# fredrikekre/PartitionedArrays.jl

Measured on AMD Instinct MI355X. Metric: SpMV+halo GB/s (frac of HBM peak), 3D Poisson 27-pt, 1/2/4/8 MI355X, higher is better.
Workload: dtype f64

## Files before the change

### include/pa_hip.h

```cpp
#ifndef PA_HIP_H
#define PA_HIP_H

#include <stdint.h>

#ifdef __cplusplus
extern "C" {
#endif

enum { PA_F32 = 0, PA_F64 = 1, PA_C64 = 2, PA_C128 = 3 };
enum { PA_REPLACE = 0, PA_ADD = 1 };

typedef struct pa_ctx pa_ctx;
typedef struct pa_index pa_index;
typedef struct pa_xchg pa_xchg;
typedef struct pa_vec pa_vec;
typedef struct pa_mat pa_mat;
typedef struct pa_coo pa_coo;

const char* pa_last_error(void);
int pa_version(void);
int pa_device_count(int* count);
int pa_tune(const char* key, int value, int* previous);
#define PA_TUNE_DROP (-2147483647 - 1)
int pa_ctx_tune(pa_ctx* c, const char* key, int value, int* previous);
// ... 22 lines not shown

int pa_xchg_create(pa_ctx* ctx,
                   int32_t n_rcv, const int32_t* parts_rcv,
                   const int32_t* ptrs_rcv, const int32_t* lids_rcv,
                   int32_t n_snd, const int32_t* parts_snd,
                   const int32_t* ptrs_snd, const int32_t* lids_snd,
                   pa_xchg** out);
int pa_xchg_destroy(pa_xchg* xg);

int pa_index_set_gids(pa_index* idx, const int64_t* lid_to_gid);
int pa_add_gids(pa_index* idx, int64_t n, const int64_t* gids, int64_t cap,
                int64_t* new_gids, int64_t* n_new);
int pa_index_to_lids(pa_index* idx, int64_t n, int64_t* ids);

int pa_vec_create(pa_ctx* ctx, int dtype, int64_t n, pa_vec** out);
int pa_vec_destroy(pa_vec* v);
int pa_vec_upload(pa_vec* v, const void* host, int64_t n);
int pa_vec_download(const pa_vec* v, void* host, int64_t n);
int pa_vec_device_ptr(const pa_vec* v, void** out);
int pa_vec_fill(pa_vec* v, const void* s);
int pa_vec_copy(pa_vec* dst, const pa_index* idx_dst,
                const pa_vec* src, const pa_index* idx_src, int same_layout);
#define PA_BCAST_F64 8
#define PA_BCAST_C128 16
int pa_vec_axpby(pa_vec* y, const pa_vec* x, const pa_index* idx,
                 const void* a, int mode, int all_lids);

int pa_mat_from_csc(pa_ctx* ctx, int dtype, int index_bytes,
                    int64_t nrows_lids, int64_t ncols_lids,
                    const void* colptr, const void* rowval, const void* nzval,
                    const pa_index* rows, const pa_index* cols,
                    pa_mat** out);
int pa_mat_from_csr(pa_ctx* ctx, int dtype, int index_bytes, int Bi,
                    int64_t nrows_lids, int64_t ncols_lids,
                    const void* rowptr, const void* colval, const void* nzval,
                    const pa_index* rows, const pa_index* cols,
                    pa_mat** out);
int pa_mat_from_coo(pa_ctx* ctx, int dtype, int index_bytes, int ids_global,
                    int64_t nrows_lids, int64_t ncols_lids, int64_t ncoo,
                    const void* I, const void* J, const void* V,
                    const pa_index* rows, const pa_index* cols,
                    int64_t* csc_nnz, int64_t* colptr_out,
                    int64_t* rowval_out, pa_mat** out);
int pa_mat_from_coo_csr(pa_ctx* ctx, int dtype, int index_bytes, int ids_global, int Bi,
                        int64_t nrows_lids, int64_t ncols_lids, int64_t ncoo,
                        const void* I, const void* J, const void* V,
                        const pa_index* rows, const pa_index* cols, int64_t* nnz,
                        int64_t* rowptr_out, int64_t* colval_out, pa_mat** out);
int pa_mat_from_dcoo_csr(const pa_coo* coo, int ids_global, int Bi, int64_t nrows_lids,
                         int64_t ncols_lids, const pa_index* rows, const pa_index* cols,
                         int64_t* nnz, int64_t* rowptr_out, int64_t* colval_out,
                         pa_mat** out);
int pa_coo_create(pa_ctx* ctx, int dtype, int64_t n, const int64_t* I,
                  const int64_t* J, const void* V, pa_coo** out);
int pa_coo_destroy(pa_coo* coo);
int pa_coo_size(const pa_coo* coo, int64_t* n);
int pa_coo_download(const pa_coo* coo, int64_t* I, int64_t* J, void* V);
int pa_coo_assemble_all(int n, pa_coo* const coo[], const pa_index* const rows[],
                        pa_xchg* const rows_xchg[]);
int pa_mat_from_dcoo(const pa_coo* coo, int ids_global, int64_t nrows_lids,
                     int64_t ncols_lids, const pa_index* rows,
                     const pa_index* cols, int64_t* csc_nnz,
                     int64_t* colptr_out, int64_t* rowval_out, pa_mat** out);
int pa_mat_set_values(pa_mat* A, const void* nzval);
int pa_mat_fillstored(pa_mat* A, const void* v);
int pa_mat_get_values(const pa_mat* A, void* nzval);
int pa_mat_xchg_create(pa_mat* A, int32_t n_rcv, const int32_t* parts_rcv,
                       const int32_t* ptrs_rcv, const int64_t* k_rcv,
                       int32_t n_snd, const int32_t* parts_snd,
                       const int32_t* ptrs_snd, const int64_t* k_snd,
                       pa_xchg** out);
int pa_mat_exchange_all(int n, pa_mat* const A[], pa_xchg* const xg[],
                        int op, int reverse, int zero_sent);
int pa_mat_destroy(pa_mat* A);
int pa_mat_info(const pa_mat* A, int64_t* nrows_owned, int64_t* nnz_owned,
                int64_t* slots, int64_t* nslices, int64_t* nslices_interior);
int pa_mat_format_info(const pa_mat* A, int64_t* pattern_slices,
                       int64_t* regular_rows, int64_t* side_rows,
                       int64_t* side_slots);
int pa_mat_delta16_info(const pa_mat* A, int64_t* delta16_slices);
int pa_mat_triple_info(const pa_mat* A, int64_t* t_slices, int64_t* t_rows, int64_t* tri_slices,
                       int64_t* tri_rows);
int pa_mat_pair_info(const pa_mat* A, int64_t* pair_slices, int64_t* pair_rows);

int pa_mat_device_ptrs(const pa_mat* A, uint64_t out[8]);

int pa_mat_traffic(const pa_mat* A, int64_t* value_bytes, int64_t* index_bytes,
                   int64_t* meta_bytes);

int pa_mat_long_rows(const pa_mat* A, int64_t* n_long, int64_t* n_long_nnz);

int pa_spmv_all(int n, pa_mat* const A[], pa_vec* const y[],
                const pa_index* const y_idx[],
                pa_vec* const x[], const pa_index* const x_idx[],
                pa_xchg* const xg[], const void* alpha, const void* beta);

int pa_spmv_dot_all(int n, pa_mat* const A[], pa_vec* const y[],
                    const pa_index* const y_idx[],
                    pa_vec* const x[], const pa_index* const x_idx[],
                    pa_xchg* const xg[], const void* alpha, const void* beta,
                    void* dot_result);
int pa_cg_update_all(int n, pa_vec* const x[], pa_vec* const r[],
                     const pa_vec* const u[], const pa_vec* const c[],
                     const pa_index* const idx[], const void* alpha,
                     double* rnorm);

int pa_cg_solve_all(int n, pa_mat* const A[], pa_vec* const x[],
                    const pa_vec* const b[], pa_vec* const u[],
                    pa_vec* const r[], pa_vec* const c[],
                    const pa_index* const idx[], pa_xchg* const xg[],
                    double reltol, double abstol, int64_t maxiter, int batch,
                    int64_t* iterations, double* residual, double* history);

typedef int (*pa_allreduce_max_fn)(float* v, int n, void* user);
int pa_cg_variant_agree(const float local_ms[2], pa_allreduce_max_fn fn, void* user, int* choice);
int pa_cg_fuse_agree(int local_can_fuse, pa_allreduce_max_fn fn, void* user, int* agreed);
int pa_mat_cg_choice(const pa_mat* A, int* choice);

int pa_exchange_all(int n, pa_vec* const v[], pa_xchg* const xg[],
                    const pa_index* const idx[], int op, int reverse,
                    int zero_ghosts);

int pa_dot_all(int n, const pa_vec* const a[], const pa_index* const ia[],
               const pa_vec* const b[], const pa_index* const ib[],
               void* result);
int pa_norm2_all(int n, const pa_vec* const a[], const pa_index* const ia[],
                 void* result);
int pa_sum_all(int n, const pa_vec* const a[], const pa_index* const ia[],
               void* result);

int pa_mat_stencil(pa_ctx* ctx, int dtype, int kind, const int64_t gdims[3],
                   const int64_t box_lo[3], const int64_t box_n[3],
                   int64_t nlids_cols, const int32_t* shell_lid,
                   const double* coeffs, int ncoeffs, pa_mat** out);

int pa_ctx_set_timing(pa_ctx* ctx, int enable);
int pa_ctx_kernel_times(pa_ctx* ctx, float* interior_ms, float* halo_ms,
                        float* boundary_ms, int* count);
int pa_ctx_last_kernel_ms(pa_ctx* ctx, float* spmv_interior_ms,
                          float* spmv_boundary_ms);
int pa_ctx_span(pa_ctx* ctx, int stop);
int pa_ctx_span_ms(pa_ctx* ctx, float* ms);

#ifdef __cplusplus
}
#endif
#endif
```

### partitionedarrays.jl_amd/_lib.py

```python
from __future__ import annotations

import ctypes as C
import os

import numpy as np

_HERE = os.path.dirname(os.path.abspath(__file__))
LIB_PATH = os.environ.get("PA_HIP_LIB") or os.path.join(_HERE, "libpa_hip.so")

PA_F32, PA_F64, PA_C64, PA_C128 = 0, 1, 2, 3
PA_REPLACE, PA_ADD = 0, 1
TUNE_DROP = -(2 ** 31)
PA_BCAST_F64, PA_BCAST_C128 = 8, 16

DTYPES = {
    np.dtype(np.float32): PA_F32,
    np.dtype(np.float64): PA_F64,
    np.dtype(np.complex64): PA_C64,
    np.dtype(np.complex128): PA_C128,
}
NP_OF = {v: k for k, v in DTYPES.items()}

_lib = None
_p = C.c_void_p
_i32p = C.POINTER(C.c_int32)
_i64p = C.POINTER(C.c_int64)

_SIGS = {
    "pa_version": [],
    "pa_device_count": [C.POINTER(C.c_int)],
    "pa_tune": [C.c_char_p, C.c_int, C.POINTER(C.c_int)],
    "pa_ctx_tune": [_p, C.c_char_p, C.c_int, C.POINTER(C.c_int)],
    "pa_knob_selftest": [C.c_int, C.c_int, C.POINTER(C.c_int)],
    "pa_cg_variant_agree": [C.POINTER(C.c_float), _p, _p, C.POINTER(C.c_int)],
    "pa_cg_fuse_agree": [C.c_int, _p, _p, C.POINTER(C.c_int)],
    "pa_mat_cg_choice": [_p, C.POINTER(C.c_int)],
    "pa_hbm_probe": [C.c_int, C.c_int64, C.c_int, C.POINTER(C.c_double), C.POINTER(C.c_double)],
    "pa_issue_stats": [C.c_int, C.POINTER(C.c_double), C.POINTER(C.c_double), C.POINTER(C.c_int64)],
    "pa_hbm_probe_launch": [C.c_int, C.c_int64, C.c_int64, C.c_int, C.POINTER(C.c_double)],
    "pa_ctx_create": [C.c_int, C.c_int, C.c_int, C.POINTER(_p)],
    "pa_ctx_create_shared": [C.c_int, C.c_int, _p, C.POINTER(_p)],
    "pa_ctx_destroy": [_p],
    "pa_ctx_sync": [_p],
    "pa_comm_unique_id": [C.c_char_p],
    "pa_comm_init_rank": [_p, C.c_char_p],
    "pa_comm_init_all": [C.c_int, C.POINTER(_p)],
    "pa_comm_stats": [_p, _i64p, _i64p],
    "pa_comm_info": [_p, C.POINTER(C.c_int), C.POINTER(C.c_int), C.POINTER(C.c_int), C.c_char_p, C.c_int,
                     C.POINTER(C.c_int), C.c_char_p, C.c_int],
    "pa_index_create": [_p, C.c_int64, C.c_int64, _i32p, C.c_int64, _i32p, C.POINTER(_p)],
    "pa_index_destroy": [_p],
    "pa_xchg_create": [_p, C.c_int32, _i32p, _i32p, _i32p, C.c_int32, _i32p, _i32p, _i32p, C.POINTER(_p)],
    "pa_xchg_destroy": [_p],
    "pa_vec_create": [_p, C.c_int, C.c_int64, C.POINTER(_p)],
    "pa_vec_destroy": [_p],
    "pa_vec_upload": [_p, _p, C.c_int64],
    "pa_vec_download": [_p, _p, C.c_int64],
    "pa_vec_device_ptr": [_p, _p],
    "pa_vec_fill": [_p, _p],
    "pa_vec_copy": [_p, _p, _p, _p, C.c_int],
    "pa_vec_axpby": [_p, _p, _p, _p, C.c_int, C.c_int],
    "pa_mat_from_csc": [_p, C.c_int, C.c_int, C.c_int64, C.c_int64, _p, _p, _p, _p, _p, C.POINTER(_p)],
    "pa_mat_from_csr": [_p, C.c_int, C.c_int, C.c_int, C.c_int64, C.c_int64, _p, _p, _p, _p, _p, C.POINTER(_p)],
    "pa_coo_create": [_p, C.c_int, C.c_int64, _i64p, _i64p, _p, C.POINTER(_p)],
    "pa_coo_destroy": [_p],
    "pa_coo_size": [_p, _i64p],
    "pa_coo_download": [_p, _i64p, _i64p, _p],
    "pa_coo_assemble_all": [C.c_int, C.POINTER(_p), C.POINTER(_p), C.POINTER(_p)],
    "pa_mat_from_dcoo": [_p, C.c_int, C.c_int64, C.c_int64, _p, _p, _i64p, _i64p, _i64p, C.POINTER(_p)],
    "pa_mat_from_coo": [_p, C.c_int, C.c_int, C.c_int, C.c_int64, C.c_int64, C.c_int64, _p, _p, _p, _p, _p, _i64p,
                        _i64p, _i64p, C.POINTER(_p)],
    "pa_mat_from_coo_csr": [_p, C.c_int, C.c_int, C.c_int, C.c_int, C.c_int64, C.c_int64, C.c_int64, _p, _p, _p, _p,
                            _p, _i64p, _i64p, _i64p, C.POINTER(_p)],
    "pa_mat_from_dcoo_csr": [_p, C.c_int, C.c_int, C.c_int64, C.c_int64, _p, _p, _i64p, _i64p, _i64p,
                             C.POINTER(_p)],
    "pa_mat_fillstored": [_p, _p],
    "pa_index_set_gids": [_p, _i64p],
    "pa_add_gids": [_p, C.c_int64, _i64p, C.c_int64, _i64p, _i64p],
    "pa_index_to_lids": [_p, C.c_int64, _i64p],
    "pa_mat_set_values": [_p, _p],
    "pa_mat_get_values": [_p, _p],
    "pa_mat_xchg_create": [_p, C.c_int32, _i32p, _i32p, _i64p, C.c_int32, _i32p, _i32p, _i64p, C.POINTER(_p)],
    "pa_mat_exchange_all": [C.c_int, C.POINTER(_p), C.POINTER(_p), C.c_int, C.c_int, C.c_int],
    "pa_mat_destroy": [_p],
    "pa_mat_info": [_p, _i64p, _i64p, _i64p, _i64p, _i64p],
    "pa_mat_format_info": [_p, _i64p, _i64p, _i64p, _i64p],
    "pa_mat_delta16_info": [_p, _i64p],
    "pa_mat_triple_info": [_p, _i64p, _i64p, _i64p, _i64p],
    "pa_mat_pair_info": [_p, _i64p, _i64p],
    "pa_mat_long_rows": [_p, _i64p, _i64p],
    "pa_mat_stencil": [_p, C.c_int, C.c_int, _i64p, _i64p, _i64p, C.c_int64, _i32p, C.POINTER(C.c_double), C.c_int, C.POINTER(_p)],
    "pa_spmv_all": [C.c_int, C.POINTER(_p), C.POINTER(_p), C.POINTER(_p), C.POINTER(_p), C.POINTER(_p), C.POINTER(_p), _p, _p],
    "pa_spmv_dot_all": [C.c_int, C.POINTER(_p), C.POINTER(_p), C.POINTER(_p), C.POINTER(_p), C.POINTER(_p), C.POINTER(_p), _p, _p, _p],
    "pa_cg_update_all": [C.c_int, C.POINTER(_p), C.POINTER(_p), C.POINTER(_p), C.POINTER(_p), C.POINTER(_p), _p, C.POINTER(C.c_double)],
    "pa_cg_solve_all": [C.c_int, C.POINTER(_p), C.POINTER(_p), C.POINTER(_p), C.POINTER(_p), C.POINTER(_p),
                        C.POINTER(_p), C.POINTER(_p), C.POINTER(_p), C.c_double, C.c_double, C.c_int64, C.c_int,
                        _i64p, C.POINTER(C.c_double), C.POINTER(C.c_double)],
    "pa_exchange_all": [C.c_int, C.POINTER(_p), C.POINTER(_p), C.POINTER(_p), C.c_int, C.c_int, C.c_int],
    "pa_dot_all": [C.c_int, C.POINTER(_p), C.POINTER(_p), C.POINTER(_p), C.POINTER(_p), _p],
    "pa_norm2_all": [C.c_int, C.POINTER(_p), C.POINTER(_p), _p],
    "pa_sum_all": [C.c_int, C.POINTER(_p), C.POINTER(_p), _p],
    "pa_ctx_last_kernel_ms": [_p, C.POINTER(C.c_float), C.POINTER(C.c_float)],
    "pa_ctx_kernel_times": [_p, C.POINTER(C.c_float), C.POINTER(C.c_float), C.POINTER(C.c_float),
                            C.POINTER(C.c_int)],
    "pa_mat_traffic": [_p, _i64p, _i64p, _i64p],
    "pa_mat_device_ptrs": [_p, _p],
    "pa_ctx_span": [_p, C.c_int],
    "pa_ctx_span_ms": [_p, C.POINTER(C.c_float)],
    "pa_ctx_set_timing": [_p, C.c_int],
}

EXPORTED = sorted(list(_SIGS) + ["pa_last_error"])


class PAError(RuntimeError):
    pass


def _prepare_runtime():
    try:
        import torch
    except Exception:
        pass


def lib():
    global _lib
    if _lib is not None:
        return _lib
    if not os.path.exists(LIB_PATH):
        raise PAError(f"{LIB_PATH} not built: run `python -c 'import __graft_entry__ as g; g.build()'`")
    _prepare_runtime()
    L = C.CDLL(LIB_PATH)
    for name, args in _SIGS.items():
        if os.environ.get("PA_HIP_LIB") and not hasattr(L, name):
            continue
        f = getattr(L, name)
        f.argtypes = args
        f.restype = C.c_int
    L.pa_last_error.argtypes = []
    L.pa_last_error.restype = C.c_char_p
    _lib = L
    return L


def call(name, *args):
    L = lib()
    rc = getattr(L, name)(*args)
    if rc != 0:
        raise PAError(f"{name}: {L.pa_last_error().decode(errors='replace')}")


def device_count() -> int:
    n = C.c_int(0)
    call("pa_device_count", C.byref(n))
    return n.value


def tune(key: str, value: int) -> int:
    prev = C.c_int(0)
    call("pa_tune", key.encode(), int(value), C.byref(prev))
    return prev.value


def knob_selftest(nthreads: int = 4, iters: int = 2000) -> int:
    n = C.c_int(-1)
    call("pa_knob_selftest", int(nthreads), int(iters), C.byref(n))
    return n.value


ALLREDUCE_MAX_FN = C.CFUNCTYPE(C.c_int, C.POINTER(C.c_float), C.c_int, C.c_void_p)

# ... 68 lines not shown
```

### partitionedarrays.jl_amd/csrc/pa_api.cpp

```cpp
#include <dlfcn.h>
#include <hip/hip_runtime.h>
#include <rccl/rccl.h>

#include <algorithm>
#include <chrono>
#include <cmath>
#include <cstdio>
#include <cstdlib>
#include <cstring>
#include <memory>
#include <numeric>
#include <string>
#include <unordered_map>
#include <atomic>
#include <condition_variable>
#include <functional>
#include <mutex>
#include <thread>
#include <vector>

#include "pa_internal.h"

namespace pa {

static thread_local std::string g_err;
void set_error(const std::string& msg) { g_err = msg; }

void launch_spmv_part(int which, int64_t nwork, const int32_t* list, const pa_mat* A, const void* x,
                      void* y, const int32_t* ymap, bool has_alpha, int bmode, const void* alpha,
                      const void* beta, void* dotp, hipStream_t st,
                      const SpmvPart* cgp = nullptr);
void launch_delta16(pa_mat* A, int64_t noids, const int32_t* kind, int32_t* ok, hipStream_t st);
void launch_pattern_detect(pa_mat* A, int64_t noids, int min_pct, int32_t* kind, int32_t* plen, int32_t* pat,
                           uint64_t* mask, int32_t* pghost, int32_t* nirreg, hipStream_t st);
void launch_side_len(pa_mat* A, int64_t n, const int32_t* rows, int32_t* len, int64_t noids,
                     int32_t* sghost, hipStream_t st);
void launch_side_fill(pa_mat* A, const int32_t* rows, const int32_t* len, hipStream_t st);
void launch_fold(int cplx, int nb, const void* in, void* scratch, void* out, unsigned* ticket, hipStream_t st);
void launch_fold_cg_alpha(int dtype, int nb, const void* in, void* scratch, void* out, unsigned* ticket,
                          CGState* cst, hipStream_t st);
void launch_fold_cg_step(int dtype, int nb, const void* in, void* scratch, void* out, unsigned* ticket,
                         CGState* cst, double* history, hipStream_t st);
void launch_cg_xr(int dtype, int64_t n, int64_t noids, const int32_t* own, void* x, void* r, const void* u,
                  const void* c, const void* alpha, const CGState* cst, double* part, int nb, hipStream_t st);
void launch_cg_xu(int dtype, int64_t n, void* x, void* u, const void* r, const CGState* cst, hipStream_t st);
void launch_cg_ghost(int dtype, int64_t lo, int64_t hi, const void* r, const void* uo, void* un, void* x,
                     const CGState* cst, hipStream_t st);
void launch_cg_alpha(int dtype, int P, const void* gathered, CGState* cst, hipStream_t st);
void launch_cg_step(int dtype, int P, const double* gathered, CGState* cst, double* history, hipStream_t st);
void launch_gather_ptrs(int P, const void* const* srcs, int accsz, void* out, hipStream_t st);
void launch_gather_scatter(int P, const void* const* srcs, int accsz, int nd, void* const* dsts, hipStream_t st);
const Knobs kDefaults = {
     223,  1,  1,  1,  1,
     65536,  2,  1,  0,  1,
     1,  0,  1,  0,  -1,  1,
     1,  1,  1,  0,  7,  1};
int coo_compress(int dtype, int index_bytes, int64_t m, int64_t ncols, int64_t n, const void* dI, const void* dJ,
                 const void* dV, int csr, int64_t* nu_out, int32_t** crow, int32_t** ccol, void** cval,
                 int64_t** colptr, hipStream_t st, hipError_t* err_out);
int coo_row_order(int64_t nu, const int32_t* crow, const int32_t* ccol, const int32_t* rl2o, const int32_t* cl2o,
                  int64_t nrows, int64_t noids_c, int64_t ncols, int H, uint64_t** key2, int64_t** idx2,
                  int64_t** rowptr, int64_t** gflag, int64_t** grank, int32_t** slen, int32_t** sghost,
                  int64_t* nnz_out, int64_t* ngh_out, hipStream_t st, hipError_t* err_out);
void coo_slices(int64_t ns, int64_t nrows, int H, const int64_t* rowptr, const uint64_t* key2, int64_t ncols,
                int64_t noids_c, const int32_t* lidx, int32_t* slen, int32_t* sghost, hipStream_t st);
void coo_fill(int dtype, int64_t nnz, int64_t nu, const uint64_t* key2, const int64_t* idx2, const int64_t* rowptr,
              const int64_t* soff, int H, int R, int64_t ncols, const int32_t* ccol, const void* cval,
              const int64_t* gflag, const int64_t* grank, int64_t slots, int32_t* col, void* val, int64_t* nz_slot,
              const int32_t* lidx, const int64_t* lptr, int32_t* lcol, int64_t long_off, hipStream_t st);
void launch_fill_i32(int64_t n, int32_t* a, int32_t v, hipStream_t st);
void launch_spmv_long(const pa_mat* A, const void* x, void* y, const int32_t* ymap, bool has_alpha, int bmode,
                      const void* alpha, const void* beta, void* dotp, int64_t dot_base, hipStream_t st);
int gid_table(int64_t n, const int64_t* d_lid_to_gid, uint64_t** sgid, int64_t** slid, hipStream_t st);
int gids_to_lids(int64_t n, int64_t* ids, const uint64_t* sgid, const int64_t* slid, int64_t nl, hipStream_t st);
int coo_assemble_pack(int dtype, int64_t n, const int64_t* I, const int64_t* J, void* V, const uint64_t* sgid,
                      const int64_t* slid, int64_t nl, const std::vector<int32_t>& lid_to_ohid, int nseg,
                      const int32_t* d_lids_rcv, const std::vector<int64_t>& ptrs_rcv, int64_t** sI, int64_t** sJ,
                      void** sV, std::vector<int64_t>* cnt, hipStream_t st);
int gids_first_touch(int64_t n, const int64_t* gids, const uint64_t* sgid, const int64_t* slid, int64_t nl,
                     int64_t** out, int64_t* m_out, hipStream_t st);
void launch_pack(int dtype, int64_t n, const int32_t* lids, const void* v, void* buf,
                 hipStream_t st, hipEvent_t ev = nullptr);
void launch_unpack(int dtype, int64_t n, const int32_t* lids, const pa_combine_plan& plan, int op,
                   const void* buf, void* v, hipStream_t st);
void launch_pull(int dtype, int64_t n, const int32_t* lids, const pa_combine_plan& plan, int op, const int32_t* bid,
                 const int64_t* elem, const void* const* bases, void* v, hipStream_t st, hipEvent_t ev = nullptr);
void launch_fill(int dtype, int64_t n, int64_t base, const int32_t* map, void* v, const void* s,
                 hipStream_t st);
int launch_spmv_merged(int n, const int* which, const SpmvPart* parts, bool has_alpha, int bmode,
                       const void* alpha, const void* beta, pa_ctx* owner,
                       hipStream_t st);
void launch_spmv_group(int which, int np, const SpmvPart* parts, bool has_alpha, int bmode, const void* alpha,
                       const void* beta, hipStream_t st);
void launch_pack_group(int dtype, const PackGroup& g, hipStream_t st);
void launch_pull_group(int dtype, const PullGroup& g, hipStream_t st);
void launch_copy(int dtype, int64_t n, const int32_t* dmap, void* d, const int32_t* smap,
                 const void* s, hipStream_t st);
void launch_axpby(int dtype, int64_t n, const int32_t* map, void* y, const void* x, const void* a,
                  int mode, hipStream_t st, int sk = 0);
void launch_reduce(int dtype, int kind, int64_t n, const int32_t* ma, const void* a,
                   const int32_t* mb, const void* b, void* partials, void* result,
                   unsigned* ticket, hipStream_t st);
void launch_stencil_count(const StencilGeom& g, const int32_t* shell, const double* coef,
                          int64_t nrows, int noids, int H, int32_t* slen, int32_t* sghost,
                          int32_t* err, hipStream_t st);
void launch_stencil_fill(const StencilGeom& g, const int32_t* shell, const double* coef,
                         int64_t nrows, int noids, pa_mat* A, int32_t* err, hipStream_t st);
void launch_probe(int copy, int unroll, int64_t n16, const void* a, void* b, int blocks, hipStream_t st);
void launch_invalid_config();
void launch_t_rowinfo(const pa_mat* A, int64_t n, const int32_t* rows, int64_t noids, int32_t* info, hipStream_t st);
void launch_t_pairinfo(const pa_mat* A, int64_t n, const int32_t* rows, int32_t* pairable, hipStream_t st);
void launch_u_fill(const pa_mat* A, hipStream_t st);
void launch_t_gbase(const pa_mat* A, int64_t noids, int32_t* ok, hipStream_t st);
void launch_t_fill(const pa_mat* A, int64_t noids, bool codes, hipStream_t st);
void launch_t_check(const pa_mat* A, unsigned* bad, hipStream_t st);

}

using namespace pa;

#define PA_FAIL(msg)             \
  do {                           \
    pa::set_error(msg);          \
    return -1;                   \
  } while (0)

#define HIPC(expr)                                                                       \
  do {                                                                                   \
    hipError_t e_ = (expr);                                                              \
    if (e_ != hipSuccess) {                                                              \
      pa::set_error(std::string(#expr) + " failed: " + hipGetErrorString(e_));           \
      return -1;                                                                         \
    }                                                                                    \
  } while (0)

#define NCCLC(expr)                                                                      \
  do {                                                                                   \
    ncclResult_t r_ = (expr);                                                            \
    if (r_ != ncclSuccess) {                                                             \
      pa::set_error(std::string(#expr) + " failed: " + ncclGetErrorString(r_));          \
      return -1;                                                                         \
    }                                                                                    \
  } while (0)

#define CHECK_ARG(cond, msg) \
  do {                       \
    if (!(cond)) PA_FAIL(msg); \
  } while (0)

namespace {

template <typename T>
int dev_upload(T** dptr, const std::vector<T>& h) {
  *dptr = nullptr;
  if (h.empty()) return 0;
  HIPC(hipMalloc((void**)dptr, h.size() * sizeof(T)));
  HIPC(hipMemcpy(*dptr, h.data(), h.size() * sizeof(T), hipMemcpyHostToDevice));
  return 0;
}

void dev_free(void* p) {
  if (p) (void)hipFree(p);
}

bool valid_dtype(int dt) { return dt == PA_F32 || dt == PA_F64 || dt == PA_C64 || dt == PA_C128; }

bool scalar_is(int dt, const void* s, double re) {
  switch (dt) {
    case PA_F32: return *(const float*)s == (float)re;
    case PA_F64: return *(const double*)s == re;
    case PA_C64: { const float* f = (const float*)s; return f[0] == (float)re && f[1] == 0.f; }
    case PA_C128: { const double* d = (const double*)s; return d[0] == re && d[1] == 0.0; }
  }
  return false;
}

int build_plan(const std::vector<int32_t>& lids, pa_combine_plan* plan) {
  const int64_t n = (int64_t)lids.size();
  std::vector<int32_t> order(n);
  std::iota(order.begin(), order.end(), 0);
  std::stable_sort(order.begin(), order.end(), [&](int32_t a, int32_t b) { return lids[a] < lids[b]; });
  std::vector<int32_t> target, ptr{0}, pos;
  pos.reserve(n);
  for (int64_t i = 0; i < n; ++i) {
    const int32_t l = lids[order[i]];
    if (target.empty() || target.back() != l) {
      if (!target.empty()) ptr.push_back((int32_t)pos.size());
      target.push_back(l);
    }
    pos.push_back(order[i]);
  }
  if (!target.empty()) ptr.push_back((int32_t)pos.size());
  plan->ntargets = (int64_t)target.size();
  plan->unique = plan->ntargets == n;
  if (!plan->unique) {
// ... 47 lines not shown
  cstart.push_back(lptr.back());
  if (dev_upload(&A->d_lchunk_start, cstart) || dev_upload(&A->d_lrow_chunk, rchunk)) return -1;
  HIPC(hipMalloc(&A->d_lpart, std::max<int64_t>(A->n_lchunks, 1) * 16));
  if (!lcol.empty() && dev_upload(&A->d_long_col, lcol)) return -1;
  return 0;
}

inline bool is_long_row(const pa_mat* A, int64_t r) {
  return A->n_long > 0 && std::binary_search(A->h_long_rows.begin(), A->h_long_rows.end(), (int32_t)r);
}

inline int64_t nvals(const pa_mat* A) { return A->slots + A->n_gnz + A->n_lnz; }

int finish_sell_layout(pa_mat* A, const std::vector<int32_t>& slen, const std::vector<char>& sghost,
                       std::vector<int64_t>* soff_out) {
  const int64_t ns = (int64_t)slen.size();
  std::vector<int64_t> soff(ns);
  int64_t acc = 0;
  for (int64_t s = 0; s < ns; ++s) {
    soff[s] = acc;
    acc += (int64_t)slen[s] * A->H;
  }
  A->slots = acc;
  A->nslices = ns;
  A->h_slen = slen;
  A->maxlen_all = 0;
  for (int32_t l : slen) A->maxlen_all = std::max(A->maxlen_all, (int)l);
  std::vector<int32_t> ilist, blist;
  for (int64_t s = 0; s < ns; ++s) (sghost[s] ? blist : ilist).push_back((int32_t)s);
  A->nslices_int = (int64_t)ilist.size();
  if (dev_upload(&A->d_slice_off, soff)) return -1;
  if (dev_upload(&A->d_slice_len, slen)) return -1;
  if (!blist.empty()) {
    if (dev_upload(&A->d_int_list, ilist)) return -1;
    if (dev_upload(&A->d_bnd_list, blist)) return -1;
  }
  if (soff_out) *soff_out = std::move(soff);
  return 0;
}

void free_uniform(pa_mat* A) {
  dev_free(A->d_uval);
  dev_free(A->d_uemap);
  A->d_uval = nullptr;
  A->d_uemap = nullptr;
  A->uK = 0;
}

int build_uniform(pa_mat* A, const std::vector<int32_t>& kind, const std::vector<int32_t>& table,
                  const std::vector<int32_t>& packed, std::vector<int32_t>& desc) {
  free_uniform(A);
  if (!knobs().spmv_uniform || A->dtype != PA_F64 || A->R != 2 || A->npatterns == 0) return 0;
  const int64_t ns = A->nslices, K0 = A->kmax, np = A->npatterns;
  std::vector<int32_t> plen(np, 0);
  for (int64_t s = 0; s < ns; ++s)
    if (kind[s] == 1) plen[packed[s] >> 9] = packed[s] & 0xff;
  std::vector<int32_t> U;
  for (int64_t p = 0; p < np; ++p)
    for (int32_t k = 0; k < plen[p]; ++k) U.push_back(table[p * K0 + k]);
  std::sort(U.begin(), U.end());
  U.erase(std::unique(U.begin(), U.end()), U.end());
  if (U.size() > 7 || U.empty()) return 0;
  const int K = (int)U.size();
  std::vector<int32_t> emap(np * 8, 0), emask(np, 0);
  for (int64_t p = 0; p < np; ++p)
    for (int32_t k = 0; k < plen[p]; ++k) {
      const int e = (int)(std::lower_bound(U.begin(), U.end(), table[p * K0 + k]) - U.begin());
      CHECK_ARG(k == 0 || e > emap[p * 8 + k - 1], "uniform layout: a pattern out of column order (internal error)");
      emap[p * 8 + k] = e;
      emask[p] |= 1 << e;
    }
  const int DW = desc_words(A->R);
  for (int64_t s = 0; s < ns; ++s)
    if (kind[s] == 1) desc[DW * s + 2] = emask[packed[s] >> 9];
  hipStream_t st = A->ctx->s_main;
  const size_t S = dtype_size(A->dtype);
  if (dev_upload(&A->d_uemap, emap)) return -1;
  HIPC(hipMalloc(&A->d_uval, (size_t)ns * A->H * K * S));
  HIPC(hipMemsetAsync(A->d_uval, 0, (size_t)ns * A->H * K * S, st));
  A->uK = K;
  for (int e = 0; e < 8; ++e) A->upat[e] = e < K ? U[e] : 0;
  launch_u_fill(A, st);
  HIPC(hipGetLastError());
  return 0;
}

int dedup_patterns(pa_mat* A, const std::vector<int32_t>& kind) {
  const int64_t ns = A->nslices, K = A->kmax;
  hipStream_t st = A->ctx->s_main;
  std::vector<int32_t> pat(ns * K);
  HIPC(hipMemcpyAsync(pat.data(), A->d_pat, ns * K * 4, hipMemcpyDeviceToHost, st));
  HIPC(hipStreamSynchronize(st));
  std::vector<int32_t> table, packed(A->h_plen);
  std::unordered_map<std::string, int32_t> ids;
  int64_t reach = 0;
  for (int64_t s = 0; s < ns; ++s) {
    if (kind[s] != 1) continue;
    const int32_t len = A->h_plen[s];
    CHECK_ARG(len >= 1 && len <= 255, "pattern slice with more than 255 entries per row");
    std::string key(reinterpret_cast<const char*>(&pat[s * K]), (size_t)len * 4);
    auto it = ids.find(key);
    int32_t id;
    if (it == ids.end()) {
      id = (int32_t)ids.size();
      CHECK_ARG(id < (1 << 22), "more than 2^22 distinct slice patterns");
      ids.emplace(std::move(key), id);
      table.insert(table.end(), pat.begin() + s * K, pat.begin() + (s + 1) * K);
      for (int32_t k = 0; k < len; ++k) reach = std::max<int64_t>(reach, std::llabs((long long)pat[s * K + k]));
    } else {
      id = it->second;
    }
    bool tri = len % 3 == 0;
    for (int32_t k = 0; tri && k < len; k += 3)
      tri = pat[s * K + k + 1] == pat[s * K + k] + 1 && pat[s * K + k + 2] == pat[s * K + k] + 2;
    packed[s] = len | ((tri ? 1 : 0) << 8) | (id << 9);
  }
  A->npatterns = (int64_t)ids.size();
  A->xcd_auto = (int)std::min<int64_t>(64, reach / (4 * A->H) / 8);
  dev_free(A->d_pat);
  A->d_pat = nullptr;
  if (table.empty()) table.assign(K, 0);
  if (dev_upload(&A->d_pat, table)) return -1;
  HIPC(hipMemcpyAsync(A->d_plen, packed.data(), ns * 4, hipMemcpyHostToDevice, st));
  {
    std::vector<int64_t> soff(ns);
    HIPC(hipMemcpyAsync(soff.data(), A->d_slice_off, ns * 8, hipMemcpyDeviceToHost, st));
    HIPC(hipStreamSynchronize(st));
    const int W = A->H / 64, DW = desc_words(A->R);
    std::vector<uint64_t> mask(ns * W);
    HIPC(hipMemcpyAsync(mask.data(), A->d_mask, ns * W * 8, hipMemcpyDeviceToHost, st));
    HIPC(hipStreamSynchronize(st));
    std::vector<int32_t> desc(DW * ns, 0);
    for (int64_t s = 0; s < ns; ++s) {
      CHECK_ARG(soff[s] % A->H == 0 && soff[s] / A->H <= INT32_MAX, "slice offset outside the descriptor's range");
      desc[DW * s] = (int32_t)(soff[s] / A->H);
      desc[DW * s + 1] = packed[s];
      std::memcpy(&desc[DW * s + 4], &mask[s * W], W * 8);
    }
    if (build_uniform(A, kind, table, packed, desc)) return -1;
    dev_free(A->d_pdesc);
    A->d_pdesc = nullptr;
    if (dev_upload(&A->d_pdesc, desc)) return -1;
  }
  HIPC(hipStreamSynchronize(st));
  return 0;
}

int remap_nz_interleaved(pa_mat* A, const std::vector<int32_t>& kind, hipStream_t st) {
  HIPC(hipStreamSynchronize(st));
  if (A->d_nz_slot) {
    A->h_nz_slot.resize(A->csc_nnz);
    HIPC(hipMemcpy(A->h_nz_slot.data(), A->d_nz_slot, A->csc_nnz * 8, hipMemcpyDeviceToHost));
    dev_free(A->d_nz_slot);
    A->d_nz_slot = nullptr;
  }
  const int64_t ns = A->nslices, R = A->R, H = A->H;
  std::vector<int64_t> soff(ns);
  HIPC(hipMemcpy(soff.data(), A->d_slice_off, ns * 8, hipMemcpyDeviceToHost));
  for (int64_t& slot : A->h_nz_slot) {
    if (slot < 0) continue;
    const int64_t s = (int64_t)(std::upper_bound(soff.begin(), soff.end(), slot) - soff.begin()) - 1;
    if (kind[s] != 3) continue;
    const int64_t t = slot - soff[s], k = t / H, w = t % H;
    slot = soff[s] + (k * 64 + w % 64) * R + w / 64;
  }
  return 0;
// ... 231 lines not shown
    HIPC(hipStreamSynchronize(st));
    dev_free(d_ok);
    int64_t nd = 0;
    for (int64_t s = 0; s < ns; ++s)
      if (ok[s]) { kind[s] = 3; ++nd; }
    if (nd == 0) {
      dev_free(A->d_col16);
      dev_free(A->d_gbase);
      A->d_col16 = nullptr;
      A->d_gbase = nullptr;
    } else {
      HIPC(hipMemcpyAsync(A->d_kind, kind.data(), ns * 4, hipMemcpyHostToDevice, st));
      if (A->nz_map && A->R == 4 && remap_nz_interleaved(A, kind, st)) return -1;
      if (knobs().spmv_tri16 && A->R <= 2 && build_triple_sell(A, kind, noids)) return -1;
    }
  }
  std::vector<int32_t> pint, pbnd, xint, xbnd, dint, dbnd, side;
  for (int64_t s = 0; s < ns; ++s) {
    if (kind[s] == 1) (pghost[s] ? pbnd : pint).push_back((int32_t)s);
    else if (kind[s] == 3) (pghost[s] ? dbnd : dint).push_back((int32_t)s);
    else if (kind[s] == 0) (pghost[s] ? xbnd : xint).push_back((int32_t)s);
    if (kind[s] == 1) {
      ++A->npattern_slices;
      const int64_t nvalid = std::min<int64_t>(A->H, A->nrows - s * A->H);
      for (int64_t i = 0; i < nvalid; ++i) {
        if ((mask[s * W + i / 64] >> (i & 63)) & 1ull) ++A->nregular_rows;
        else if (!is_long_row(A, s * A->H + i)) side.push_back((int32_t)(s * A->H + i));
      }
    }
  }
  A->h_kind = kind;
  A->maxlen_pat = A->maxlen_pm_int = A->maxlen_d16 = 0;
  for (int64_t s = 0; s < ns; ++s) {
    if (kind[s] == 1) A->maxlen_pat = std::max(A->maxlen_pat, (int)A->h_plen[s]);
    else if (kind[s] == 0) A->maxlen_pm_int = std::max(A->maxlen_pm_int, (int)A->h_slen[s]);
    else if (kind[s] == 3) A->maxlen_d16 = std::max(A->maxlen_d16, (int)A->h_slen[s]);
  }
  A->np_int = (int64_t)pint.size();
  A->np_bnd = (int64_t)pbnd.size();
  A->nx_int = (int64_t)xint.size();
  A->nx_bnd = (int64_t)xbnd.size();
  A->nd_int = (int64_t)dint.size();
  A->nd_bnd = (int64_t)dbnd.size();
  if (dev_upload(&A->d_pint_list, pint) || dev_upload(&A->d_pbnd_list, pbnd) ||
      dev_upload(&A->d_xint_list, xint) || dev_upload(&A->d_xbnd_list, xbnd) ||
      dev_upload(&A->d_dint_list, dint) || dev_upload(&A->d_dbnd_list, dbnd))
    return -1;
  A->s_nrows = (int64_t)side.size();
  std::vector<int32_t> rl;
  if (A->s_nrows > 0) {
    if (dev_upload(&A->d_s_rowmap, side)) return -1;
    int32_t* srow = A->d_s_rowmap;
    int32_t* d_dummy = nullptr;
    A->s_nslices = (A->s_nrows + A->H - 1) / A->H;
    HIPC(hipMalloc((void**)&A->d_s_rowlen, A->s_nrows * 4));
    HIPC(hipMalloc((void**)&d_dummy, A->s_nslices * 4));
    HIPC(hipMemsetAsync(d_dummy, 0, A->s_nslices * 4, st));
    launch_side_len(A, A->s_nrows, srow, A->d_s_rowlen, noids, d_dummy, st);
    HIPC(hipGetLastError());
    rl.resize(A->s_nrows);
    HIPC(hipMemcpyAsync(rl.data(), A->d_s_rowlen, A->s_nrows * 4, hipMemcpyDeviceToHost, st));
    HIPC(hipStreamSynchronize(st));
    dev_free(d_dummy);
  }
  if (A->s_nrows > 0) {
    int32_t* srow = A->d_s_rowmap;
    std::vector<int32_t> slen(A->s_nslices, 0);
    std::vector<int64_t> soff(A->s_nslices);
    for (int64_t i = 0; i < A->s_nrows; ++i) slen[i / A->H] = std::max(slen[i / A->H], rl[i]);
    A->maxlen_side = 0;
    for (int32_t l : slen) A->maxlen_side = std::max(A->maxlen_side, (int)l);
    int64_t acc = 0;
    for (int64_t s = 0; s < A->s_nslices; ++s) { soff[s] = acc; acc += (int64_t)slen[s] * A->H; }
    A->s_slots = acc;
    if (dev_upload(&A->d_s_off, soff) || dev_upload(&A->d_s_len, slen)) return -1;
    const size_t S = dtype_size(A->dtype);
    HIPC(hipMalloc((void**)&A->d_s_col, std::max<int64_t>(acc, 1) * 4));
    HIPC(hipMalloc(&A->d_s_val, std::max<int64_t>(acc, 1) * S));
    launch_side_fill(A, srow, A->d_s_rowlen, st);
    HIPC(hipGetLastError());
    HIPC(hipStreamSynchronize(st));
  }
  A->has_pat = true;
  return 0;
}

struct LocalSet {
  std::vector<int> pos_of_part;
  int find(int part) const {
    return (part >= 1 && part < (int)pos_of_part.size()) ? pos_of_part[part] : -1;
  }
};

template <typename H>
LocalSet local_set(int n, H* const* hs) {
  LocalSet L;
  int maxp = 0;
  bool all_comm = true;
  for (int i = 0; i < n; ++i) {
    const pa_ctx* c = hs[i]->ctx;
    maxp = std::max(maxp, c->nparts);
    all_comm = all_comm && c->comm != nullptr && (c->halo_rccl || knobs().halo_transport == 1);
  }
  L.pos_of_part.assign(maxp + 1, -1);
  if (all_comm) return L;
  for (int i = 0; i < n; ++i) L.pos_of_part[hs[i]->ctx->part] = i;
  return L;
}

uint64_t g_xchg_next_id = 1;

int build_pull(int i, int n, pa_xchg* const xg[], const LocalSet& L, int dtype, int dir, bool alt = false) {
  pa_xchg* X = xg[i];
  pa_ctx* c = X->ctx;
  pa_pull& P = alt ? X->pull_alt : X->pull[dir];
  auto sender_buf = [&](const pa_xchg* Q) -> void* {
    return alt ? Q->d_buf_snd2 : (dir == 0 ? Q->d_buf_snd : Q->d_buf_rcv);
  };
  const auto& prcv = dir == 0 ? X->parts_rcv : X->parts_snd;
  const auto& orcv = dir == 0 ? X->ptrs_rcv : X->ptrs_snd;
  void* own = dir == 0 ? X->d_buf_rcv : X->d_buf_snd;
  std::vector<const void*> key;
  key.push_back((const void*)(intptr_t)dtype_size(dtype));
  for (int32_t q : prcv) {
    const int j = L.find(q);
    key.push_back(j >= 0 ? (const void*)(uintptr_t)xg[j]->id : nullptr);
    key.push_back(j >= 0 ? sender_buf(xg[j]) : own);
  }
  if (P.built && P.key == key) return 0;
  dev_free(P.d_bid);
  dev_free(P.d_elem);
  dev_free(P.d_bases);
  P = pa_pull{};
  P.built = true;
  P.key = key;
  HIPC(hipSetDevice(c->device));
  std::vector<void*> bases;
  auto base_id = [&](void* b) {
    for (size_t t = 0; t < bases.size(); ++t)
      if (bases[t] == b) return (int32_t)t;
    bases.push_back(b);
    return (int32_t)(bases.size() - 1);
  };
  const int64_t nslots = orcv.empty() ? 0 : orcv.back();
  std::vector<int32_t> bid(nslots);
  std::vector<int64_t> elem(nslots);
  for (size_t k = 0; k < prcv.size(); ++k) {
    const int j = L.find(prcv[k]);
    const int64_t cnt = orcv[k + 1] - orcv[k];
    if (j < 0) {
      const int32_t b = base_id(own);
      for (int64_t t = 0; t < cnt; ++t) { bid[orcv[k] + t] = b; elem[orcv[k] + t] = orcv[k] + t; }
      continue;
    }
    pa_xchg* Q = xg[j];
    const auto& qsnd = dir == 0 ? Q->parts_snd : Q->parts_rcv;
    const auto& qo = dir == 0 ? Q->ptrs_snd : Q->ptrs_rcv;
    int m = -1;
    for (size_t t = 0; t < qsnd.size(); ++t)
      if (qsnd[t] == c->part) { m = (int)t; break; }
    CHECK_ARG(m >= 0, "exchanger mismatch: a receiver lists a sender that does not send to it");
    CHECK_ARG(cnt == qo[m + 1] - qo[m], "exchanger mismatch: segment lengths differ (SequentialBackend.jl:187)");
    const int qdev = Q->ctx->device;
    if (qdev != c->device) {
      int can = 0;
      HIPC(hipDeviceCanAccessPeer(&can, c->device, qdev));
// ... 374 lines not shown
  const Knobs* kn_ = nullptr;
  int n_ = 0;
  std::vector<std::thread> workers_;
};

}

static std::shared_ptr<void> own_comm(ncclComm_t comm) {
  return std::shared_ptr<void>((void*)comm, [](void* p) { (void)ncclCommDestroy((ncclComm_t)p); });
}

extern "C" {

const char* pa_last_error(void) { return g_err.c_str(); }
int pa_version(void) { return 1; }

}
namespace {
struct Knob {
  const char* key;
  int Knobs::*slot;
  int64_t Knobs::*slot64;
  int64_t lo, hi;
  int64_t mask;
  const char* help;
};
const Knob kKnobs[] = {
    {"spmv_flags", &Knobs::spmv_flags, nullptr, 0, 0xff, 0xff,
     "spmv_flags: bit 0 = non-temporal streams, bit 1 = pattern and triple-SELL slices' one-load descriptor, "
     "bit 2 = 16 B x runs (pattern rows), bit 3 = masked tail batch, bit 4 = identity slice lists dropped, "
     "bit 5 = non-temporal y stores, bit 6 = short-row kernels (launches whose rows have <= 8 entries), "
     "bit 7 = the Float64 short-row tail launch at 7 entries and 7 waves per SIMD (rows <= 7 entries)"},
    {"long_rows_exact", &Knobs::long_exact, nullptr, 0, 1, 0,
     "long_rows_exact: 1 = reference summation order, 0 = lane-strided tree (1e-12)"},
    {"halo_pull", &Knobs::halo_pull, nullptr, 0, 1, 0,
     "halo_pull: 1 = receivers read the senders' buffers (one kernel), 0 = staging copies"},
    {"spmv_delta16", &Knobs::spmv_delta16, nullptr, 0, 1, 0,
     "spmv_delta16: 1 = int32-column slices whose columns fit 16-bit codes store those (matrices built "
     "afterwards; default), 0 = int32 column ids"},
    {"spmv_merge", &Knobs::spmv_merge, nullptr, 0, 1, 0,
     "spmv_merge: 1 = mul! without a halo in flight (one part, or parts of one stream pair with the direct "
     "pull) runs every slice kind of every part as one launch (default), 0 = one launch per kind"},
    {"spmv_merge_max", nullptr, &Knobs::spmv_merge_max, 0, INT32_MAX, 0,
     "spmv_merge_max: one part with more slices than this runs one launch per kind (0: always merge)"},
    {"cg_fuse", &Knobs::cg_fuse, nullptr, 0, 2, 0,
     "cg_fuse: 1 = the device CG computes u = r .+ beta.*u inside the SpMV, 0 = a separate sweep, "
     "2 = auto (default: one batch of each, then the faster; all parts in one process, else the sweep)"},
    {"halo_direct", &Knobs::halo_direct, nullptr, 0, 1, 0,
     "halo_direct: 1 = mul! over parts sharing a stream pair reads the ghosts straight from the owners' x "
     "on the compute stream (default), 0 = pack + pull on the comm stream"},
    {"halo_transport", &Knobs::halo_transport, nullptr, 0, 1, 0,
     "halo_transport: 0 = parts of this process by device reads/copies, 1 = RCCL send/recv for every part "
     "with a communicator (pa_comm_init_all)"},
    {"spmv_group", &Knobs::spmv_group, nullptr, 0, 1, 0,
     "spmv_group: 1 = one launch per phase for parts sharing a stream pair, 0 = per part"},
    {"spmv_format", &Knobs::spmv_format, nullptr, 0, 1, 0, "spmv_format: 0 = int32 columns, 1 = pattern slices"},
    {"pattern_min_regular", &Knobs::pattern_min_pct, nullptr, 0, 100, 0,
     "pattern_min_regular: a slice becomes a pattern slice when at least this % of its rows follow its pattern "
     "(matrices built afterwards); 0 = auto (default): 70 for 128-row slices, 50 for Float32's 256-row slices"},
    {"issue_threads", &Knobs::issue_threads, nullptr, 0, 2, 0,
     "issue_threads: a call over parts with their own stream pairs is issued from host threads, one part "
     "per thread: 1 = when the parts span several devices (default), 2 = always, 0 = never (the calling "
     "thread, one part after the other)"},
    {"spmv_tri16", &Knobs::spmv_tri16, nullptr, 0, 1, 0,
     "spmv_tri16: the delta16 slices' rows re-sliced into the triple SELL (rows of consecutive column triples "
     "keep one 16-bit code per triple; matrices built afterwards): 1 = slices of 1-2 rows per lane (Float64, "
     "ComplexF32, ComplexF64, Float32 with f32_rows 2; default), 0 = never"},
    {"f32_rows", &Knobs::f32_rows, nullptr, 0, 4, 6,
     "f32_rows: Float32 SELL rows per lane (matrices built afterwards): 4 = 16 B value packs in 256-row "
     "slices, 2 = 8 B packs in 128-row slices (the Float64 geometry; delta16 rows then take the triple "
     "SELL), 0 = auto (default): 4, rebuilt with 2 when fewer than 80 % of the slices are pattern slices "
     "(C5 F32 -7 %, FE27 256^3 F32 +14 % with 2, profiles/r05/af/)"},
    {"spmv_tri_pack", &Knobs::tri_pack, nullptr, 0, 7, 0,
     "spmv_tri_pack: triple-SELL slices of 2 rows per lane (matrices built afterwards): bit 2 = pair slices "
     "(all element types): rows a, a + 1 whose columns differ by one, entry for entry, share one lane, one "
     "code and one x run per triple (C5 F32 -2.4 %, F64 -1 %, profiles/r06/u/); bit 0 = Float32 pair slices: "
     "a triple's values as one 16 B pack (entries 0 and 1 of both rows) and one 8 B pack (entry 2) per lane "
     "(two loads instead of three); bit 1: unused since r06/aa (the Float32 tri slices' code packs); 7 = "
     "default, 0 = none"},
    {"spmv_uniform", &Knobs::spmv_uniform, nullptr, 0, 1, 0,
     "spmv_uniform: Float64 pattern slices whose patterns (<= 7 entries) fit one union U (FD7; matrices built "
     "afterwards): 1 = a copy of their values at slice * H * |U| in U's entry order, so the short-row tail "
     "launch issues its value and x loads before the slice descriptor arrives (default), 0 = off"},
    {"spmv_side_tail", &Knobs::side_tail, nullptr, 0, 1, 0,
     "spmv_side_tail: per-kind launches without a halo in flight (big single parts): 1 = the side rows (<= 8 "
     "entries) run as the trailing waves of the pattern launch (default: FE27 256^3 -0.4 %, profiles/r05/o/), "
     "0 = a launch of their own after it"},
    {"spmv_tri_order", &Knobs::tri_order, nullptr, 0, 1, 0,
     "spmv_tri_order: the triple SELL's row order (matrices built afterwards): 1 = the other rows first "
     "(their slower waves start early, the launch ends on uniform triple slices; default: C5 F64 -1 %, "
     "Float32 triples -4..-7 %, profiles/r05/n/), 0 = rows of column triples first"},
    {"halo_barrier", &Knobs::halo_barrier, nullptr, 0, 2, 0,
     "halo_barrier: mul! over parts with their own stream pairs and local neighbours (one process driving "
     "several GPUs): 1 = one pack barrier event per call and double-buffered send buffers (default), 2 = the "
     "same with each part's pull on its compute stream after its interior slices (one runtime call less per "
     "part), 0 = per-neighbour event waits before every pack and every pull"},
    {"spmv_xcd_chunk", &Knobs::spmv_xcd_chunk, nullptr, -1, 64, 0,
     "spmv_xcd_chunk: the SpMV launches' workgroups in runs of C consecutive blocks per XCD (C > 0; the x lines "
     "of neighbouring slices shared in one L2), 0 = the hardware's round robin, -1 = auto (default): per-kind "
     "launches (big single parts) take C = the pattern's reach in blocks / 8, so that a block's z-neighbour "
     "plane runs on its XCD (FE27 256^3 F64: C = 16, -1.0..-1.2 %, profiles/r05/q,r/), merged launches keep "
     "the round robin (C2: C = 4 +1.4 %, r05/k/)"},
    {"fault_inject", &Knobs::fault_inject, nullptr, 0, 1, 0,
     "fault_inject: 1 = every job of a threaded issue (IssuePool) also issues an invalid kernel launch (tests "
     "of the error path; test_exception.jl's role), 0 = off (default)"},
};
constexpr int kNumKnobs = (int)(sizeof(kKnobs) / sizeof(kKnobs[0]));
static_assert(kNumKnobs <= pa_ctx::kMaxKnobs, "pa_ctx::over too small");

std::mutex g_knob_mu;
Knobs g_knob_defaults = kDefaults;
thread_local const Knobs* t_knobs = nullptr;
thread_local Knobs t_knob_snapshot;

int knob_find(const char* key) {
  for (int i = 0; i < kNumKnobs; ++i)
    if (!std::strcmp(key, kKnobs[i].key)) return i;
  pa::set_error(std::string("pa_tune: unknown key ") + key);
  return -1;
}
int knob_index(const char* key, int64_t value) {
  const int i = knob_find(key);
  if (i < 0) return -1;
  const Knob& k = kKnobs[i];
  if (value < k.lo || value > k.hi || (k.mask != 0 && (value & ~k.mask) != 0)) {
    pa::set_error(k.help);
    return -2;
  }
  return i;
}
int64_t knob_get(const Knobs& K, int i) { return kKnobs[i].slot ? (int64_t)(K.*kKnobs[i].slot) : K.*kKnobs[i].slot64; }
void knob_set(Knobs& K, int i, int64_t v) {
  if (kKnobs[i].slot) K.*kKnobs[i].slot = (int)v;
  else K.*kKnobs[i].slot64 = v;
}
}

namespace pa {
const Knobs& knobs() {
  if (t_knobs) return *t_knobs;
  std::lock_guard<std::mutex> g(g_knob_mu);
  t_knob_snapshot = g_knob_defaults;
  return t_knob_snapshot;
}
KnobBind::KnobBind(const Knobs* k) : prev(t_knobs) { t_knobs = k; }
KnobBind::~KnobBind() { t_knobs = prev; }
thread_local int t_force_f32_rows = 0;
int f32_rows_knob() { return t_force_f32_rows ? t_force_f32_rows : (knobs().f32_rows == 2 ? 2 : 4); }
struct ForceF32Rows {
  int prev;
  explicit ForceF32Rows(int r) : prev(t_force_f32_rows) { t_force_f32_rows = r; }
  ~ForceF32Rows() { t_force_f32_rows = prev; }
};
}

TuneScope::TuneScope(const pa_ctx* c) : prev(t_knobs) {
  if (prev) {
    k = *prev;
  } else {
    std::lock_guard<std::mutex> g(g_knob_mu);
    k = g_knob_defaults;
  }
  if (c && !prev)
    for (int i = 0; i < kNumKnobs; ++i)
      if (c->has_over[i]) knob_set(k, i, c->over[i]);
  t_knobs = &k;
// ... 1302 lines not shown
      const int64_t k = std::find(qr.begin(), qr.end(), c->part) - qr.begin();
      const Side& src = sd[jj];
      const int64_t from = src.off[k];
      const int sdev = xg[jj]->ctx->device;
      if (sdev == c->device) {
        HIPC(hipMemcpyAsync(d.nI + at, src.sI + from, m * 8, hipMemcpyDeviceToDevice, c->s_main));
        HIPC(hipMemcpyAsync(d.nJ + at, src.sJ + from, m * 8, hipMemcpyDeviceToDevice, c->s_main));
        HIPC(hipMemcpyAsync((char*)d.nV + at * S, (const char*)src.sV + from * S, m * S, hipMemcpyDeviceToDevice,
                            c->s_main));
      } else {
        HIPC(hipMemcpyPeerAsync(d.nI + at, c->device, src.sI + from, sdev, m * 8, c->s_main));
        HIPC(hipMemcpyPeerAsync(d.nJ + at, c->device, src.sJ + from, sdev, m * 8, c->s_main));
        HIPC(hipMemcpyPeerAsync((char*)d.nV + at * S, c->device, (const char*)src.sV + from * S, sdev, m * S,
                                c->s_main));
      }
    }
    for (size_t k = 0; k < X->parts_rcv.size(); ++k) {
      const int64_t m = d.cnt[k];
      const int q = X->parts_rcv[k];
      if (m == 0 || L.find(q) >= 0) continue;
      const int pr = c->peer_rank(q);
      ncclComm_t cm = (ncclComm_t)c->comm;
      ops.push_back({c->part, q, true, (char*)(d.sI + d.off[k]), (size_t)m * 8, pr, cm, c->s_main});
      ops.push_back({c->part, q, true, (char*)(d.sJ + d.off[k]), (size_t)m * 8, pr, cm, c->s_main});
      ops.push_back({c->part, q, true, (char*)d.sV + d.off[k] * S, (size_t)m * S, pr, cm, c->s_main});
    }
  }
  if (!ops.empty() && rccl_group(ops)) { free_all(); return -1; }
  for (int i = 0; i < n; ++i) {
    HIPC(hipSetDevice(coo[i]->ctx->device));
    HIPC(hipStreamSynchronize(coo[i]->ctx->s_main));
  }
  for (int i = 0; i < n; ++i) {
    pa_coo* C = coo[i];
    Side& d = sd[i];
    HIPC(hipSetDevice(C->ctx->device));
    dev_free(C->d_I);
    dev_free(C->d_J);
    dev_free(C->d_V);
    C->d_I = d.nI;
    C->d_J = d.nJ;
    C->d_V = d.nV;
    C->n = d.nn;
    d.nI = nullptr;
    d.nJ = nullptr;
    d.nV = nullptr;
  }
  free_all();
  return 0;
}

static int load_nz_map(const pa_mat* cA) {
  CHECK_ARG(cA->nz_map, "matrix was not built from a CSC pattern");
  pa_mat* A = const_cast<pa_mat*>(cA);
  if (A->d_nz_slot) {
    HIPC(hipSetDevice(A->ctx->device));
    HIPC(hipStreamSynchronize(A->ctx->s_main));
    A->h_nz_slot.resize(A->csc_nnz);
    HIPC(hipMemcpy(A->h_nz_slot.data(), A->d_nz_slot, A->csc_nnz * 8, hipMemcpyDeviceToHost));
    dev_free(A->d_nz_slot);
    A->d_nz_slot = nullptr;
  }
  return 0;
}

static inline int64_t nz_index(const pa_mat* A, int64_t p) {
  const int64_t s = A->h_nz_slot[p];
  return s >= 0 ? s : A->slots - s - 1;
}

static int refresh_side(pa_mat* A, hipStream_t st) {
  if (A->s_nrows > 0) {
    launch_side_fill(A, A->d_s_rowmap, A->d_s_rowlen, st);
    HIPC(hipGetLastError());
  }
  if (A->t_nrows > 0) {
    launch_t_fill(A, 0, false, st);
    HIPC(hipGetLastError());
  }
  if (A->d_uval) {
    launch_u_fill(A, st);
    HIPC(hipGetLastError());
  }
  return 0;
}

int pa_mat_set_values(pa_mat* A, const void* nzval) {
  CHECK_ARG(A && nzval, "null argument");
  if (load_nz_map(A)) return -1;
  HIPC(hipSetDevice(A->ctx->device));
  const size_t S = dtype_size(A->dtype);
  const int64_t nv = nvals(A);
  std::vector<unsigned char> hval(nv * S, 0);
  for (int64_t p = 0; p < A->csc_nnz; ++p)
    std::memcpy(&hval[nz_index(A, p) * S], (const unsigned char*)nzval + p * S, S);
  HIPC(hipStreamSynchronize(A->ctx->s_main));
  if (nv) HIPC(hipMemcpy(A->d_val, hval.data(), nv * S, hipMemcpyHostToDevice));
  if (refresh_side(A, A->ctx->s_main)) return -1;
  HIPC(hipStreamSynchronize(A->ctx->s_main));
  return 0;
}

int pa_mat_fillstored(pa_mat* A, const void* v) {
  CHECK_ARG(A && v, "null argument");
  HIPC(hipSetDevice(A->ctx->device));
  const int64_t nv = nvals(A);
  if (nv) launch_fill(A->dtype, nv, 0, nullptr, A->d_val, v, A->ctx->s_main);
  HIPC(hipGetLastError());
  if (refresh_side(A, A->ctx->s_main)) return -1;
  return 0;
}

int pa_mat_get_values(const pa_mat* A, void* nzval) {
  CHECK_ARG(A && nzval, "null argument");
  if (load_nz_map(A)) return -1;
  HIPC(hipSetDevice(A->ctx->device));
  const size_t S = dtype_size(A->dtype);
  const int64_t nv = nvals(A);
  std::vector<unsigned char> hval(nv * S, 0);
  HIPC(hipStreamSynchronize(A->ctx->s_comm));
  HIPC(hipStreamSynchronize(A->ctx->s_main));
  if (nv) HIPC(hipMemcpy(hval.data(), A->d_val, nv * S, hipMemcpyDeviceToHost));
  for (int64_t p = 0; p < A->csc_nnz; ++p)
    std::memcpy((unsigned char*)nzval + p * S, &hval[nz_index(A, p) * S], S);
  return 0;
}

int pa_mat_xchg_create(pa_mat* A, int32_t n_rcv, const int32_t* parts_rcv, const int32_t* ptrs_rcv,
                       const int64_t* k_rcv, int32_t n_snd, const int32_t* parts_snd, const int32_t* ptrs_snd,
                       const int64_t* k_snd, pa_xchg** out) {
  CHECK_ARG(A && out, "null argument");
  if (load_nz_map(A)) return -1;
  CHECK_ARG(nvals(A) < ((int64_t)1 << 31), "matrix exchanger: value index exceeds int32");
  CHECK_ARG(n_rcv >= 0 && n_snd >= 0, "negative neighbour count");
  auto conv = [&](int32_t n, const int32_t* ptrs, const int64_t* k, std::vector<int32_t>& o) -> int {
    const int64_t m = n > 0 ? (int64_t)ptrs[n] - 1 : 0;
    CHECK_ARG(m >= 0, "matrix exchanger: bad ptrs");
    o.resize(m);
    for (int64_t i = 0; i < m; ++i) {
      CHECK_ARG(k[i] >= 1 && k[i] <= A->csc_nnz, "matrix exchanger: nz index out of range");
      o[i] = (int32_t)(nz_index(A, k[i] - 1) + 1);
    }
    return 0;
  };
  std::vector<int32_t> lr, ls;
  if (conv(n_rcv, ptrs_rcv, k_rcv, lr) || conv(n_snd, ptrs_snd, k_snd, ls)) return -1;
  return pa_xchg_create(A->ctx, n_rcv, parts_rcv, ptrs_rcv, lr.data(), n_snd, parts_snd, ptrs_snd, ls.data(),
                        out);
}

int pa_mat_exchange_all(int n, pa_mat* const A[], pa_xchg* const xg[], int op, int reverse, int zero_sent) {
  CHECK_ARG(n >= 1 && A && xg && A[0], "null argument");
  TuneScope ts(A[0]->ctx);
  std::vector<pa_vec> vs(n);
  std::vector<pa_vec*> vp(n);
  for (int i = 0; i < n; ++i) {
    CHECK_ARG(A[i] && xg[i] && A[i]->ctx == xg[i]->ctx, "exchange!(A): matrix and exchanger of different parts");
    vs[i].ctx = A[i]->ctx;
    vs[i].dtype = A[i]->dtype;
    vs[i].n = nvals(A[i]);
    vs[i].d = A[i]->d_val;
    vp[i] = &vs[i];
  }
  if (pa_exchange_all(n, vp.data(), xg, nullptr, op, reverse, 0)) return -1;
  for (int i = 0; i < n; ++i) {
    pa_ctx* c = A[i]->ctx;
    HIPC(hipSetDevice(c->device));
    if (zero_sent) {
      unsigned char z[16] = {0};
      if (reverse) launch_fill(A[i]->dtype, xg[i]->n_rcv_data, 0, xg[i]->d_lids_rcv, A[i]->d_val, z, c->s_main);
      else launch_fill(A[i]->dtype, xg[i]->n_snd_data, 0, xg[i]->d_lids_snd, A[i]->d_val, z, c->s_main);
    }
    if (refresh_side(A[i], c->s_main)) return -1;
  }
  HIPC(hipGetLastError());
  return 0;
}

int pa_mat_destroy(pa_mat* A) {
  if (!A) return 0;
  (void)hipSetDevice(A->ctx->device);
  (void)hipStreamSynchronize(A->ctx->s_main);
  dev_free(A->d_slice_off);
  dev_free(A->d_slice_len);
  dev_free(A->d_int_list);
  dev_free(A->d_bnd_list);
  dev_free(A->d_col);
  dev_free(A->d_val);
  dev_free(A->d_nz_slot);
  for (void* p : {(void*)A->d_kind, (void*)A->d_plen, (void*)A->d_pdesc, (void*)A->d_pat, (void*)A->d_mask,
                  (void*)A->d_pint_list, (void*)A->d_pbnd_list, (void*)A->d_xint_list,
                  (void*)A->d_xbnd_list, (void*)A->d_s_off, (void*)A->d_s_len,
                  (void*)A->d_s_col, A->d_s_val, (void*)A->d_s_rowmap, (void*)A->d_s_rowlen, A->d_dotp,
                  (void*)A->d_long_row, (void*)A->d_long_ptr, (void*)A->d_long_col, (void*)A->d_sflags,
                  (void*)A->d_lmask, (void*)A->d_lchunk_start, (void*)A->d_lrow_chunk, A->d_lpart,
                  (void*)A->d_col16, (void*)A->d_gbase, (void*)A->d_dint_list, (void*)A->d_dbnd_list})
    dev_free(p);
  free_triple_sell(A);
  free_uniform(A);
  delete A;
  return 0;
}

int pa_mat_format_info(const pa_mat* A, int64_t* pattern_slices, int64_t* regular_rows,
                       int64_t* side_rows, int64_t* side_slots) {
  CHECK_ARG(A, "null matrix");
  if (pattern_slices) *pattern_slices = A->npattern_slices;
  if (regular_rows) *regular_rows = A->nregular_rows;
  if (side_rows) *side_rows = A->s_nrows;
  if (side_slots) *side_slots = A->s_slots;
  return 0;
}

int pa_mat_delta16_info(const pa_mat* A, int64_t* delta16_slices) {
  CHECK_ARG(A, "null matrix");
  if (delta16_slices) *delta16_slices = A->nd_int + A->nd_bnd;
  return 0;
}

int pa_mat_pair_info(const pa_mat* A, int64_t* pair_slices, int64_t* pair_rows) {
  CHECK_ARG(A, "null matrix");
  if (pair_slices) *pair_slices = A->t_pair_slices;
  if (pair_rows) *pair_rows = A->t_pair_rows;
  return 0;
}

int pa_mat_triple_info(const pa_mat* A, int64_t* t_slices, int64_t* t_rows, int64_t* tri_slices,
                       int64_t* tri_rows) {
  CHECK_ARG(A, "null matrix");
  if (t_slices) *t_slices = A->t_nslices;
  if (t_rows) *t_rows = A->t_nrows;
  if (tri_slices) *tri_slices = A->t_tri_slices;
  if (tri_rows) *tri_rows = A->t_tri_rows;
  return 0;
}

int pa_mat_long_rows(const pa_mat* A, int64_t* n_long, int64_t* n_long_nnz) {
  CHECK_ARG(A, "null matrix");
  if (n_long) *n_long = A->n_long;
  if (n_long_nnz) *n_long_nnz = A->n_lnz;
  return 0;
}

int pa_mat_device_ptrs(const pa_mat* A, uint64_t out[8]) {
  CHECK_ARG(A && out, "null argument");
  const void* p[8] = {A->d_val, A->d_col, A->d_slice_off, A->d_plen, A->d_pat, A->d_mask, A->d_s_val, A->d_s_col};
  for (int i = 0; i < 8; ++i) out[i] = (uint64_t)(uintptr_t)p[i];
  return 0;
}

int pa_mat_traffic(const pa_mat* A, int64_t* value_bytes, int64_t* index_bytes, int64_t* meta_bytes) {
  CHECK_ARG(A, "null matrix");
  TuneScope ts(A->ctx);
  const int64_t S = (int64_t)dtype_size(A->dtype), H = A->H, W = H / 64;
  const bool pat = knobs().spmv_format == 1 && A->has_pat;
  const bool split = A->d_bnd_list != nullptr;
  int64_t v = 0, ix = 0, m = 0;
  for (int64_t s = 0; s < A->nslices; ++s) {
    const int kd = pat ? A->h_kind[s] : 0;
    if (kd == 1) {
      v += (int64_t)(A->d_uval ? A->uK : A->h_plen[s]) * H * S;
      m += std::max<int64_t>(W * 8 + 8 + 4, 4 * desc_words(A->R)) + 4;
    } else if (kd == 3) {
      v += (int64_t)A->h_slen[s] * H * S;
      ix += (int64_t)A->h_slen[s] * H * 2;
      m += 8 + 4 + 4 + 4;
    } else if (kd == 5) {
    } else {
      v += (int64_t)A->h_slen[s] * H * S;
      ix += (int64_t)A->h_slen[s] * H * 4;
      m += 8 + 4 + ((pat || split) ? 4 : 0);
    }
  }
  if (pat) {
    m += A->npatterns * A->kmax * 4;
    v += A->s_slots * S;
    ix += A->s_slots * 4 + A->s_nrows * 4;
    m += A->s_nslices * 12;
    v += A->t_slots * S;
    ix += A->t_code_slots * 2 + A->t_nrows * 4;
    m += A->t_nslices * (8 + 4 + 4 + 4);
  }
  v += A->n_lnz * S;
  ix += A->n_lnz * 4;
  m += A->n_long * 16;
  if (value_bytes) *value_bytes = v;
  if (index_bytes) *index_bytes = ix;
  if (meta_bytes) *meta_bytes = m;
  return 0;
}

int pa_mat_info(const pa_mat* A, int64_t* nrows, int64_t* nnz, int64_t* slots, int64_t* nslices,
                int64_t* nslices_int) {
  CHECK_ARG(A, "null matrix");
  if (nrows) *nrows = A->nrows;
  if (nnz) *nnz = A->nnz;
  if (slots) *slots = A->slots;
  if (nslices) *nslices = A->nslices;
  if (nslices_int) *nslices_int = A->nslices_int;
  return 0;
}

constexpr int kMaxTimed = 1024;

struct CGFuse {
  std::vector<const void*> u_old;
  std::vector<void*> u_new, xacc;
  std::vector<CGState*> st;
};

static void cg_ghosts(const CGFuse* fz, int i, const pa_mat* A, const pa_vec* r, hipStream_t st) {
  if (!fz || r->n <= A->nrows) return;
  launch_cg_ghost(A->dtype, A->nrows, r->n, r->d, fz->u_old[i], fz->u_new[i], fz->xacc[i], fz->st[i], st);
}

static int group_ok(int n, pa_mat* const A[], pa_xchg* const xg[], bool any_x, int dt) {
  if (!knobs().spmv_group || (n < 2 && any_x)) return 0;
  const pa_ctx* c0 = A[0]->ctx;
  for (int i = 0; i < n; ++i)
    if (A[i]->ctx->s_main != c0->s_main || A[i]->ctx->s_comm != c0->s_comm) return 0;
  if (!any_x) return 1;
  if (!knobs().halo_pull) return 0;
  LocalSet L = local_set(n, xg);
  for (int i = 0; i < n; ++i)
    for (const auto* lst : {&xg[i]->parts_snd, &xg[i]->parts_rcv})
      for (int32_t q : *lst)
        if (L.find(q) < 0) return 0;
  for (int i = 0; i < n; ++i)
    if (!xg[i]->plan_fwd.unique) return 0;
  if (knobs().halo_direct) {
    bool ok = true;
    for (int i = 0; i < n && ok; ++i) {
      if (build_direct(i, n, xg, L)) return 0;
      ok = xg[i]->direct.ok;
    }
    if (ok) return 2;
  }
  for (int i = 0; i < n; ++i) {
    if (build_pull(i, n, xg, L, dt, 0)) return 0;
    if (!xg[i]->pull[0].ok) return 0;
  }
  return 1;
}
// ... 1148 lines not shown
```

### partitionedarrays.jl_amd/csrc/pa_internal.h

```cpp
#pragma once
#include <hip/hip_runtime.h>
#include <cstdint>
#include <memory>
#include <string>
#include <vector>

#include "../../include/pa_hip.h"

namespace pa {

struct alignas(8) c64 {
  float re, im;
};
struct alignas(16) c128 {
  double re, im;
};

__host__ __device__ inline c64 operator+(c64 a, c64 b) { return {a.re + b.re, a.im + b.im}; }
__host__ __device__ inline c64 operator-(c64 a, c64 b) { return {a.re - b.re, a.im - b.im}; }
__host__ __device__ inline c64 operator*(c64 a, c64 b) {
  return {a.re * b.re - a.im * b.im, a.re * b.im + a.im * b.re};
}
__host__ __device__ inline c128 operator+(c128 a, c128 b) { return {a.re + b.re, a.im + b.im}; }
__host__ __device__ inline c128 operator-(c128 a, c128 b) { return {a.re - b.re, a.im - b.im}; }
// ... 185 lines not shown
  int np;
  int64_t n[PA_GROUP_MAX];
  const int32_t* lids[PA_GROUP_MAX];
  const void* v[PA_GROUP_MAX];
  void* buf[PA_GROUP_MAX];
};
struct PullGroup {
  int np;
  int64_t n[PA_GROUP_MAX];
  const int32_t* lids[PA_GROUP_MAX];
  const int32_t* bid[PA_GROUP_MAX];
  const int64_t* elem[PA_GROUP_MAX];
  const void* const* bases[PA_GROUP_MAX];
  void* v[PA_GROUP_MAX];
};

struct StencilGeom {
  int64_t N[3];
  int64_t lo[3];
  int64_t n[3];
  int kind;
};

}

struct pa_ctx {
  struct StreamRefs { int n = 1; };
  StreamRefs* stream_refs = nullptr;
  int device = 0;
  int part = 1;
  int nparts = 1;
  hipStream_t s_main = nullptr;
  hipStream_t s_comm = nullptr;
  void* comm = nullptr;
  bool halo_rccl = false;
  std::shared_ptr<void> comm_owner;
  std::shared_ptr<const std::vector<int>> rank_of_part;
  int peer_rank(int q) const { return rank_of_part ? (*rank_of_part)[q - 1] : q - 1; }
  int64_t rccl_bytes_sent = 0, rccl_bytes_recv = 0;
  void* d_partials = nullptr;
  void* d_fold = nullptr;
  void* d_result = nullptr;
  void* d_gather = nullptr;
  unsigned* d_ticket = nullptr;
  void* h_pinned = nullptr;
  bool timing = false;
  std::vector<hipEvent_t> tev;
  int tn = 0;
  hipEvent_t span_ev[2] = {nullptr, nullptr};
  hipEvent_t ev_packed = nullptr;
  hipEvent_t ev_recvd = nullptr;
  hipEvent_t ev_barrier = nullptr;
  std::vector<std::pair<std::vector<void*>, void**>> bases_cache;
  std::vector<std::pair<std::vector<char>, void*>> merged_cache;
  static constexpr int kMaxKnobs = 24;
  bool has_over[kMaxKnobs] = {};
  int64_t over[kMaxKnobs] = {};
};

namespace pa {
struct Knobs {
  int spmv_flags;
  int long_exact;
  int halo_pull;
  int spmv_delta16;
  int spmv_merge;
  int64_t spmv_merge_max;
  int cg_fuse;
  int halo_direct;
  int halo_transport;
  int spmv_group;
  int spmv_format;
  int pattern_min_pct;
  int issue_threads;
  int fault_inject;
  int spmv_xcd_chunk;
  int spmv_tri16;
  int halo_barrier;
  int tri_order;
  int side_tail;
  int f32_rows;
  int tri_pack;
  int spmv_uniform;
};
const Knobs& knobs();
struct KnobBind {
  explicit KnobBind(const Knobs* k);
  ~KnobBind();
  const Knobs* prev;
};
}

struct TuneScope {
  explicit TuneScope(const pa_ctx* c);
  ~TuneScope();
  TuneScope(const TuneScope&) = delete;
  TuneScope& operator=(const TuneScope&) = delete;
  pa::Knobs k;
  const pa::Knobs* prev;
};

struct pa_index {
  pa_ctx* ctx = nullptr;
  int64_t nlids = 0, noids = 0, nhids = 0;
  bool own_contig = true;
  bool ghost_contig = true;
  int32_t* d_oid_to_lid = nullptr;
  int32_t* d_hid_to_lid = nullptr;
  std::vector<int32_t> h_oid_to_lid;
  std::vector<int32_t> h_hid_to_lid;
  std::vector<int32_t> h_lid_to_ohid;
  uint64_t* d_sgid = nullptr;
  int64_t* d_slid = nullptr;
  bool has_gids = false;
};

struct pa_combine_plan {
  int64_t ntargets = 0;
  bool unique = true;
  int32_t* d_target = nullptr;
  int32_t* d_ptr = nullptr;
  int32_t* d_pos = nullptr;
};

struct pa_pull {
  bool built = false;
  bool ok = false;
  std::vector<const void*> key;
  int32_t* d_bid = nullptr;
  int64_t* d_elem = nullptr;
  void** d_bases = nullptr;
  std::vector<int32_t> h_bid;
  std::vector<int64_t> h_elem;
  std::vector<void*> h_bases;
};

struct pa_xchg {
  pa_ctx* ctx = nullptr;
  uint64_t id = 0;
  pa_pull pull[2];
  pa_pull direct;
  std::vector<int32_t> h_lids_snd;
  std::vector<int32_t> parts_rcv, parts_snd;
  std::vector<int64_t> ptrs_rcv, ptrs_snd;
  int64_t n_rcv_data = 0, n_snd_data = 0;
  int64_t max_lid = -1;
  int32_t* d_lids_rcv = nullptr;
  int32_t* d_lids_snd = nullptr;
  void* d_buf_rcv = nullptr;
  void* d_buf_snd = nullptr;
  void* d_buf_snd2 = nullptr;
  pa_pull pull_alt;
  uint64_t fast_key = 0, fast_seq = 0;
  int fast_parity = 0;
  pa_combine_plan plan_fwd;
  pa_combine_plan plan_rev;
};

constexpr size_t kVecPad = 64;

struct pa_coo {
  pa_ctx* ctx = nullptr;
  int dtype = PA_F64;
  int64_t n = 0;
  int64_t* d_I = nullptr;
  int64_t* d_J = nullptr;
// ... 10 lines not shown

constexpr int desc_words(int R) { return R <= 2 ? 8 : 16; }

struct pa_mat {
  pa_ctx* ctx = nullptr;
  int dtype = PA_F64;
  int cg_fuse_choice = -1;
  int R = 2;
  int H = 128;
  int64_t nrows = 0;
  int64_t ncols_lids = 0;
  int64_t nnz = 0;
  int64_t slots = 0;
  int64_t nslices = 0;
  int64_t nslices_int = 0;
  bool csr = false;
  std::vector<int32_t> h_slen;
  std::vector<int32_t> h_kind;
  std::vector<int32_t> h_plen;
  int maxlen_all = INT32_MAX, maxlen_pm_int = INT32_MAX, maxlen_pat = INT32_MAX, maxlen_side = INT32_MAX;
  int64_t* d_slice_off = nullptr;
  int32_t* d_slice_len = nullptr;
  int32_t* d_int_list = nullptr;
  int32_t* d_bnd_list = nullptr;
  int32_t* d_col = nullptr;
  void* d_val = nullptr;
  std::vector<int64_t> h_nz_slot;
  int64_t* d_nz_slot = nullptr;
  bool nz_map = false;
  int64_t csc_nnz = 0;
  int64_t n_gnz = 0;
  int64_t n_long = 0, n_lnz = 0, long_off = 0;
  int32_t* d_long_row = nullptr;
  int64_t* d_long_ptr = nullptr;
  int32_t* d_long_col = nullptr;
  int32_t* d_sflags = nullptr;
  uint64_t* d_lmask = nullptr;
  std::vector<int32_t> h_long_rows;
  int64_t n_lchunks = 0;
  int64_t* d_lchunk_start = nullptr;
  int64_t* d_lrow_chunk = nullptr;
  void* d_lpart = nullptr;

  bool has_pat = false;
  int kmax = 0;
  int32_t* d_kind = nullptr;
  int32_t* d_pdesc = nullptr;
  int32_t* d_plen = nullptr;
  int32_t* d_pat = nullptr;
  int64_t npatterns = 0;
  int xcd_auto = 0;
  uint64_t* d_mask = nullptr;
  int32_t* d_pint_list = nullptr;
  int32_t* d_pbnd_list = nullptr;
  int64_t np_int = 0, np_bnd = 0;
  int32_t* d_xint_list = nullptr;
  int32_t* d_xbnd_list = nullptr;
  int64_t nx_int = 0, nx_bnd = 0;
  int64_t npattern_slices = 0, nregular_rows = 0;
  uint16_t* d_col16 = nullptr;
  int32_t* d_gbase = nullptr;
  int32_t* d_dint_list = nullptr;
  int32_t* d_dbnd_list = nullptr;
  int64_t nd_int = 0, nd_bnd = 0;
  int maxlen_d16 = INT32_MAX;
  int64_t s_nrows = 0, s_nslices = 0, s_slots = 0;
  int64_t* d_s_off = nullptr;
  int32_t* d_s_len = nullptr;
  int32_t* d_s_col = nullptr;
  void* d_s_val = nullptr;
  int32_t* d_s_rowmap = nullptr;
  int32_t* d_s_rowlen = nullptr;
  int64_t t_nrows = 0, t_nslices = 0, t_slots = 0, t_tri_slices = 0, t_tri_rows = 0, t_code_slots = 0;
  int64_t* d_t_off = nullptr;
  int32_t* d_t_len = nullptr;
  uint16_t* d_t_col16 = nullptr;
  void* d_t_val = nullptr;
  int t_pack = 0;
  int64_t t_pair_slices = 0, t_pair_rows = 0;
  void* d_uval = nullptr;
  int32_t* d_uemap = nullptr;
  int uK = 0;
  int32_t upat[8] = {0, 0, 0, 0, 0, 0, 0, 0};
  int32_t* d_t_gbase = nullptr;
  int32_t* d_t_desc = nullptr;
  int32_t* d_t_rowmap = nullptr;
  int64_t* d_t_src = nullptr;
  int32_t* d_t_rowlen = nullptr;
  int32_t* d_t_int_list = nullptr;
  int32_t* d_t_bnd_list = nullptr;
  int64_t nt_int = 0, nt_bnd = 0;
  int maxlen_t = INT32_MAX;
  std::vector<int32_t> h_t_len;
  void* d_dotp = nullptr;
};
```

### partitionedarrays.jl_amd/csrc/pa_spmv.hip

```cpp
#include "pa_internal.h"

#include <cstddef>

#include <algorithm>
#include <cstring>
#include <type_traits>

#if defined(PA_SPMV_DT)
#define PA_DT_DEFINE 0
#else
#define PA_DT_DEFINE 1
#endif
#define PA_CAT2(a, b) a##b
#define PA_CAT(a, b) PA_CAT2(a, b)

namespace pa {

template <typename T, int R>
struct alignas(sizeof(T) * R) Pack {
  T v[R];
};
template <int R>
struct alignas(4 * R) IPack {
  int32_t c[R];
};
template <int R>
struct alignas(2 * R) S16Pack {
  uint16_t c[R];
};

enum { SPMV_NT = 1, SPMV_DESC = 2 , SPMV_XPAIR = 4, SPMV_TAILB = 8, SPMV_IDLIST = 16, SPMV_YNT = 32, SPMV_SHORT = 64,
       SPMV_SHORT7 = 128 ,
       SPMV_PRODA = 256 ,
       SPMV_TPACK = 512  };

typedef unsigned int spmv_u32x4 __attribute__((ext_vector_type(4)));
static_assert((SPMV_NT | SPMV_DESC | SPMV_XPAIR | SPMV_TAILB | SPMV_IDLIST | SPMV_SHORT | SPMV_SHORT7) == 223,
              "kDefaults.spmv_flags");
template <int R>
constexpr int kDescWords = desc_words(R);

#if defined(__HIP_DEVICE_COMPILE__)
#define PA_GLB __attribute__((address_space(1)))
#else
#define PA_GLB
#endif

template <int BYTES> struct RawOf;
template <> struct RawOf<2> { typedef unsigned short type; };
template <> struct RawOf<4> { typedef unsigned int type; };
template <> struct RawOf<8> { typedef unsigned int type __attribute__((ext_vector_type(2))); };
template <> struct RawOf<16> { typedef unsigned int type __attribute__((ext_vector_type(4))); };

template <bool NT, typename V>
__device__ __forceinline__ V ld(const V* p) {
  typedef typename RawOf<sizeof(V)>::type Raw;
  Raw r;
  if (NT) r = __builtin_nontemporal_load(reinterpret_cast<const Raw*>(p));
  else r = *reinterpret_cast<const Raw*>(p);
  V v;
  __builtin_memcpy(&v, &r, sizeof(V));
  return v;
}

template <typename T>
struct SpmvArgs {
  int64_t nwork;
  const PA_GLB int32_t* list;
  const PA_GLB int64_t* soff;
  const PA_GLB int32_t* slen;
  const PA_GLB int32_t* col;
  const PA_GLB T* val;
  const PA_GLB int32_t* pat;
  const PA_GLB uint64_t* mask;
  int kmax;
  const PA_GLB int32_t* rowmap;
  int64_t nrows;
  const PA_GLB T* x;
  int64_t nx;
  PA_GLB T* y;
  const PA_GLB int32_t* ymap;
  T alpha, beta;
  int flags;
  const PA_GLB T* dotu;
  void* dotp;
  int64_t dot_base;
  const PA_GLB int32_t* sflags;
  const PA_GLB uint64_t* lmask;
  int maxlen;
  const PA_GLB uint16_t* col16;
  const PA_GLB int32_t* gbase;
  const PA_GLB int32_t* ilv;
  const PA_GLB T* xu;
  PA_GLB T* un;
  PA_GLB T* xacc;
  const PA_GLB CGState* cg;
  int xcd_chunk;
  const PA_GLB int32_t* desc;
  const PA_GLB T* uval;
  int uK;
  int32_t upat[8];
};

template <typename T> struct DAcc { using type = double; };
template <> struct DAcc<c64> { using type = c128; };
template <> struct DAcc<c128> { using type = c128; };
__device__ inline double dacc(float a) { return (double)a; }
__device__ inline double dacc(double a) { return a; }
__device__ inline c128 dacc(c64 a) { return c128{(double)a.re, (double)a.im}; }
__device__ inline c128 dacc(c128 a) { return a; }
__device__ inline double shfl_down_acc(double v, int d) { return __shfl_down(v, d, 64); }
__device__ inline c128 shfl_down_acc(c128 v, int d) {
  return c128{__shfl_down(v.re, d, 64), __shfl_down(v.im, d, 64)};
}

__device__ __forceinline__ float pick(bool c, float a, float b) { return c ? a : b; }
__device__ __forceinline__ double pick(bool c, double a, double b) { return c ? a : b; }
__device__ __forceinline__ c64 pick(bool c, c64 a, c64 b) { return c64{c ? a.re : b.re, c ? a.im : b.im}; }
__device__ __forceinline__ c128 pick(bool c, c128 a, c128 b) { return c128{c ? a.re : b.re, c ? a.im : b.im}; }

typedef unsigned int u4a __attribute__((ext_vector_type(4))) __attribute__((aligned(4)));
typedef unsigned int u2r __attribute__((ext_vector_type(2))) __attribute__((aligned(4)));
template <typename T, int R>
__device__ __forceinline__ Pack<T, R> ld_xrun(const T* p) {
  Pack<T, R> v;
  if constexpr (sizeof(Pack<T, R>) == 8) {
    const u2r r = *reinterpret_cast<const u2r*>(p);
    __builtin_memcpy(&v, &r, 8);
  } else {
    static_assert(sizeof(Pack<T, R>) == 16, "16 B runs");
    const u4a r = *reinterpret_cast<const u4a*>(p);
    __builtin_memcpy(&v, &r, 16);
  }
  return v;
}

typedef unsigned int u3a __attribute__((ext_vector_type(3))) __attribute__((aligned(4)));
typedef unsigned int u2a __attribute__((ext_vector_type(2))) __attribute__((aligned(4)));
template <typename T>
__device__ __forceinline__ void ld_xtrip(const T* p, T (&o)[3]) {
  if constexpr (sizeof(T) == 4) {
    const u3a r = *reinterpret_cast<const u3a*>(p);
    __builtin_memcpy(&o[0], &r, 12);
  } else if constexpr (sizeof(T) == 8) {
    const u4a r = *reinterpret_cast<const u4a*>(p);
    const u2a q = *reinterpret_cast<const u2a*>(p + 2);
    __builtin_memcpy(&o[0], &r, 16);
    __builtin_memcpy(&o[2], &q, 8);
  } else {
#pragma unroll
    for (int j = 0; j < 3; ++j) o[j] = p[j];
  }
}

template <typename T>
__device__ __forceinline__ void ld_xquad(const T* p, T (&o)[4]) {
  if constexpr (sizeof(T) == 4) {
    const u4a r = *reinterpret_cast<const u4a*>(p);
    __builtin_memcpy(&o[0], &r, 16);
  } else if constexpr (sizeof(T) == 8) {
    const u4a r0 = *reinterpret_cast<const u4a*>(p);
    const u4a r1 = *reinterpret_cast<const u4a*>(p + 2);
    __builtin_memcpy(&o[0], &r0, 16);
    __builtin_memcpy(&o[2], &r1, 16);
  } else {
#pragma unroll
    for (int j = 0; j < 4; ++j) o[j] = p[j];
  }
}

template <typename T, bool XV>
struct XSrc {
  const T* __restrict__ x;
  __device__ __forceinline__ T get(int64_t j) const { return x[j]; }
  __device__ __forceinline__ void quad(int64_t j, T (&o)[4]) const { ld_xquad<T>(x + j, o); }
  template <int R>
  __device__ __forceinline__ Pack<T, R> run(int64_t j) const { return ld_xrun<T, R>(x + j); }
  __device__ __forceinline__ void trip(int64_t j, T (&o)[3]) const { ld_xtrip<T>(x + j, o); }
};
template <typename T>
struct XSrc<T, true> {
  const T* __restrict__ r;
  const T* __restrict__ u;
  double b;
// ... 333 lines not shown
    q[0] = ld<NT>(&cp[t * 64]);
#pragma unroll
    for (int u = 0; u < 3; ++u) v[u] = ld<NT>(&vp[(3 * t + u) * 64]);
    step(q, v, std::integral_constant<int, 1>{});
  }
}

template <typename T, bool ALPHA, typename XS, bool TP, int NB, bool FULL>
__device__ __forceinline__ void pair_batch(T (&acc)[2], const uint16_t* __restrict__ cs,
                                           const Pack<T, 2>* __restrict__ vp, int t, int ntri, const XS& x, T alpha,
                                           bool pf, int32_t rowa, int32_t gb, bool packs) {
  constexpr int R = 2, NQ = NB / 4;
  const int lane = threadIdx.x % 64;
  uint16_t q[NB];
  if (FULL && packs) {
    const uint16_t* __restrict__ cb = cs + (int64_t)t * 64;
#pragma unroll
    for (int h = 0; h < NQ; ++h) {
      const S16Pack<4> q4 = ld<true>(reinterpret_cast<const S16Pack<4>*>(cb + h * 4 * 64) + lane);
#pragma unroll
      for (int i = 0; i < 4; ++i) q[4 * h + i] = q4.c[i];
    }
#pragma unroll
    for (int u = 4 * NQ; u < NB; ++u) q[u] = ld<true>(reinterpret_cast<const S16Pack<1>*>(cb + u * 64) + lane).c[0];
  } else {
#pragma unroll
    for (int u = 0; u < NB; ++u)
      q[u] = ld<true>(reinterpret_cast<const S16Pack<1>*>(cs + (int64_t)(FULL ? t + u : min(t + u, ntri - 1)) * 64) +
                      lane).c[0];
  }
  Pack<T, R> v[3 * NB];
  const Pack<T, R>* __restrict__ vb = vp - lane;
#pragma unroll
  for (int u = 0; u < NB; ++u) {
    const int tu = FULL ? t + u : min(t + u, ntri - 1);
    if constexpr (TP) {
      const Pack<T, R>* tb = vb + (int64_t)tu * 3 * 64;
      const Pack<T, 2 * R> p01 = ld<true>(reinterpret_cast<const Pack<T, 2 * R>*>(tb) + lane);
#pragma unroll
      for (int r = 0; r < R; ++r) {
        v[3 * u].v[r] = p01.v[r];
        v[3 * u + 1].v[r] = p01.v[R + r];
      }
      v[3 * u + 2] = ld<true>(tb + 2 * 64 + lane);
    } else {
#pragma unroll
      for (int j = 0; j < 3; ++j) v[3 * u + j] = ld<true>(&vp[(3 * tu + j) * 64]);
    }
  }
  T xq[NB][4];
  bool ok[NB];
#pragma unroll
  for (int u = 0; u < NB; ++u) {
    const int32_t c = d16_col(q[u], rowa, gb);
    ok[u] = c >= 0 && (FULL || t + u < ntri);
    x.quad(c >= 0 ? c : 0, xq[u]);
  }
#pragma unroll
  for (int u = 0; u < NB; ++u)
#pragma unroll
    for (int j = 0; j < 3; ++j) {
      const T t0 = acc[0] + term<ALPHA>(v[3 * u + j].v[0], xq[u][j], alpha, pf);
      const T t1 = acc[1] + term<ALPHA>(v[3 * u + j].v[1], xq[u][j + 1], alpha, pf);
      acc[0] = pick(ok[u], t0, acc[0]);
      acc[1] = pick(ok[u], t1, acc[1]);
    }
}

template <typename T, bool ALPHA, typename XS, bool TP>
__device__ __forceinline__ void rows_t16_pair(T (&acc)[2], const uint16_t* __restrict__ cs,
                                              const Pack<T, 2>* __restrict__ vp, int len, const XS& x, T alpha,
                                              bool pf, int32_t rowa, int32_t gb) {
  constexpr int B = sizeof(T) == 4 ? 9 : kTriBatch;
  const int ntri = len / 3;
  int t = 0;
  for (; t + B <= ntri; t += B) pair_batch<T, ALPHA, XS, TP, B, true>(acc, cs, vp, t, ntri, x, alpha, pf, rowa, gb, true);
  if constexpr (sizeof(T) == 4) {
    if (t < ntri) pair_batch<T, ALPHA, XS, TP, B, false>(acc, cs, vp, t, ntri, x, alpha, pf, rowa, gb, false);
  } else {
    for (; t < ntri; ++t) pair_batch<T, ALPHA, XS, TP, 1, true>(acc, cs, vp, t, ntri, x, alpha, pf, rowa, gb, false);
  }
}

template <typename T, int R, bool ALPHA, bool NT, int U, bool XP, bool SH = false, typename XS>
__device__ __forceinline__ void rows_pattern(T (&acc)[R], const int32_t* __restrict__ pat,
                                             const Pack<T, R>* __restrict__ vp, int len,
                                             const XS& x, int64_t rbase,
                                             const bool (&ok)[R], T alpha, bool pf, bool TB) {
  if (SH) TB = true;
  int64_t xb[R];
  bool any = false;
#pragma unroll
  for (int r = 0; r < R; ++r) {
    xb[r] = ok[r] ? rbase + r : -1;
    any = any || ok[r];
  }
  int k = 0;
  for (; !SH && k + U <= len; k += U) {
    int32_t o[U];
    Pack<T, R> v[U];
#pragma unroll
    for (int u = 0; u < U; ++u) o[u] = pat[k + u];
#pragma unroll
    for (int u = 0; u < U; ++u) v[u] = ld<NT>(&vp[(k + u) * 64]);
    T xv[U][R];
    if constexpr (XP && R > 1) {
#pragma unroll
      for (int u = 0; u < U; ++u) {
        const Pack<T, R> xr = x.template run<R>(any ? rbase + o[u] : 0);
#pragma unroll
        for (int r = 0; r < R; ++r) xv[u][r] = xr.v[r];
      }
    } else {
#pragma unroll
      for (int u = 0; u < U; ++u)
#pragma unroll
        for (int r = 0; r < R; ++r) xv[u][r] = x.get(xb[r] >= 0 ? xb[r] + o[u] : 0);
    }
#pragma unroll
    for (int u = 0; u < U; ++u)
#pragma unroll
      for (int r = 0; r < R; ++r) {
        acc[r] = acc[r] + term<ALPHA>(v[u].v[r], xv[u][r], alpha, pf);
      }
  }
  if (TB && k < len) {
    int32_t o[U];
    Pack<T, R> v[U];
#pragma unroll
    for (int u = 0; u < U; ++u) o[u] = pat[min(k + u, len - 1)];
#pragma unroll
    for (int u = 0; u < U; ++u)
      if (k + u < len) v[u] = ld<NT>(&vp[(k + u) * 64]);
    T xv[U][R];
    if constexpr (XP && R > 1) {
#pragma unroll
      for (int u = 0; u < U; ++u)
        if (k + u < len) {
          const Pack<T, R> xr = x.template run<R>(any ? rbase + o[u] : 0);
#pragma unroll
          for (int r = 0; r < R; ++r) xv[u][r] = xr.v[r];
        }
    } else {
#pragma unroll
      for (int u = 0; u < U; ++u)
        if (k + u < len)
#pragma unroll
          for (int r = 0; r < R; ++r) xv[u][r] = x.get(xb[r] >= 0 ? xb[r] + o[u] : 0);
    }
#pragma unroll
    for (int u = 0; u < U; ++u)
      if (k + u < len) {
#pragma unroll
        for (int r = 0; r < R; ++r) {
          acc[r] = acc[r] + term<ALPHA>(v[u].v[r], xv[u][r], alpha, pf);
        }
      }
    k = len;
  }
  for (; !SH && k < len; ++k) {
    const int32_t o = pat[k];
    const Pack<T, R> v = ld<NT>(&vp[k * 64]);
#pragma unroll
    for (int r = 0; r < R; ++r) {
      acc[r] = acc[r] + term<ALPHA>(v.v[r], x.get(xb[r] >= 0 ? xb[r] + o : 0), alpha, pf);
    }
  }
}

template <typename T, int R, bool ALPHA, bool NT, typename XS>
__device__ __forceinline__ void rows_pattern_tri(T (&acc)[R], const int32_t* __restrict__ pat,
                                                 const Pack<T, R>* __restrict__ vp, int len, const XS& x,
                                                 int64_t rbase, const bool (&ok)[R], T alpha, bool pf) {
  static_assert(R > 1, "runs of R > 1 values");
  bool any = false;
#pragma unroll
  for (int r = 0; r < R; ++r) any = any || ok[r];
  auto triple = [&](int32_t o, T (&xv)[3][R]) {
    Pack<T, R> A, B;
    if constexpr (R == 2 && sizeof(T) == 4) {
      T q[4];
      x.quad(any ? rbase + o : 0, q);
      A.v[0] = q[0];
      A.v[1] = q[1];
      B.v[0] = q[2];
      B.v[1] = q[3];
    } else {
      A = x.template run<R>(any ? rbase + o : 0);
      B = x.template run<R>(any ? rbase + o + 2 : 0);
    }
#pragma unroll
    for (int r = 0; r < R; ++r) {
      xv[0][r] = A.v[r];
      xv[1][r] = r + 1 < R ? A.v[r + 1] : B.v[R - 2];
      xv[2][r] = B.v[r];
    }
  };
  int k = 0;
  constexpr int TB = kTriBatch;
  for (; k + 3 * TB <= len; k += 3 * TB) {
    int32_t o[TB];
#pragma unroll
    for (int t = 0; t < TB; ++t) o[t] = pat[k + 3 * t];
    Pack<T, R> v[3 * TB];
#pragma unroll
    for (int u = 0; u < 3 * TB; ++u) v[u] = ld<NT>(&vp[(k + u) * 64]);
    T xv[TB][3][R];
#pragma unroll
    for (int t = 0; t < TB; ++t) triple(o[t], xv[t]);
#pragma unroll
    for (int t = 0; t < TB; ++t)
#pragma unroll
      for (int j = 0; j < 3; ++j)
#pragma unroll
        for (int r = 0; r < R; ++r) acc[r] = acc[r] + term<ALPHA>(v[3 * t + j].v[r], xv[t][j][r], alpha, pf);
  }
  for (; k < len; k += 3) {
    const int32_t o = pat[k];
    Pack<T, R> v[3];
#pragma unroll
    for (int j = 0; j < 3; ++j) v[j] = ld<NT>(&vp[(k + j) * 64]);
    T xv[3][R];
    triple(o, xv);
#pragma unroll
    for (int j = 0; j < 3; ++j)
#pragma unroll
      for (int r = 0; r < R; ++r) acc[r] = acc[r] + term<ALPHA>(v[j].v[r], xv[j][r], alpha, pf);
  }
}

template <typename W> __device__ inline W cg_alpha_of(const CGState* st);
template <> __device__ inline double cg_alpha_of<double>(const CGState* st) { return st->alpha.re; }
template <> __device__ inline c128 cg_alpha_of<c128>(const CGState* st) { return st->alpha; }

template <typename T, int R, bool UPD, typename XS, typename W>
__device__ __forceinline__ void cg_rows_update(const SpmvArgs<T>& a, const XS& xs, int64_t i0, int rs, W alpha,
                                               bool xpend = true, T* unv = nullptr) {
  T* xacc = (T*)a.xacc;
  T* un = (T*)a.un;
  if (rs == 1 && i0 + R <= a.nrows) {
    const Pack<T, R> uo = *reinterpret_cast<const Pack<T, R>*>(xs.u + i0);
    if (UPD) {
      const Pack<T, R> rv = *reinterpret_cast<const Pack<T, R>*>(xs.r + i0);
      Pack<T, R> o;
#pragma unroll
      for (int k = 0; k < R; ++k) o.v[k] = xs.f(rv.v[k], uo.v[k]);
      *reinterpret_cast<Pack<T, R>*>(un + i0) = o;
#pragma unroll
      for (int k = 0; k < R; ++k) unv[k] = o.v[k];
    }
    if (xpend) {
      Pack<T, R> xv = ld<true>(reinterpret_cast<const Pack<T, R>*>(xacc + i0));
#pragma unroll
      for (int k = 0; k < R; ++k) xv.v[k] = narrow<T>(widen(xv.v[k]) + alpha * widen(uo.v[k]));
      if constexpr (sizeof(Pack<T, R>) == 16) {
        spmv_u32x4 w;
        __builtin_memcpy(&w, &xv, 16);
        __builtin_nontemporal_store(w, reinterpret_cast<spmv_u32x4*>(xacc + i0));
      } else {
        *reinterpret_cast<Pack<T, R>*>(xacc + i0) = xv;
      }
    }
    return;
  }
#pragma unroll
  for (int k = 0; k < R; ++k) {
    const int64_t i = i0 + (int64_t)k * rs;
    if (i >= a.nrows) {
      if (UPD) unv[k] = zero_of<T>();
      continue;
    }
    const T uo = xs.u[i];
    if (UPD) {
      unv[k] = xs.f(xs.r[i], uo);
      un[i] = unv[k];
    }
    if (xpend) xacc[i] = narrow<T>(widen(xacc[i]) + alpha * widen(uo));
  }
}

template <typename T, int R, bool ALPHA, int BMODE, int U, int PK, bool SH = false, bool XV = false>
__device__ __forceinline__ void spmv_wave(const SpmvArgs<T>& a, const int64_t w) {
  constexpr bool PAT = PK == 1;
  constexpr int H = 64 * R;
  const int lane = threadIdx.x & 63;
  const int64_t s = a.list ? (int64_t)a.list[w] : w;
  bool il = false;
  if constexpr (PK == 3) il = kInterleaveD16<R>;
  if constexpr (PK == 4) il = true;
  if constexpr (PK == 0 && kInterleaveD16<R>) il = a.ilv && a.ilv[s] == 3;
  const int rs = il ? 64 : 1;
  const int64_t row0 = s * H + (il ? (int64_t)lane : (int64_t)lane * R);
  XSrc<T, XV> xs;
  bool xpend = false, main_rows = false;
  typename wide_of<T>::type xalpha{};
  if constexpr (XV) {
    const CGState* cg = (const CGState*)a.cg;
    xpend = cg->it > cg->xit;
    xalpha = cg_alpha_of<typename wide_of<T>::type>(cg);
    xs.r = (const T*)a.x;
    xs.u = (const T*)a.xu;
    xs.b = (cg->res * cg->res) / (cg->prev * cg->prev);
    main_rows = a.rowmap == nullptr;
    if (cg->done) {
      if (xpend && main_rows) cg_rows_update<T, R, false>(a, xs, row0, rs, xalpha);
      return;
    }
  } else {
    xs.x = (const T*)a.x;
  }
  int64_t off;
  int32_t lraw;
  uint64_t dmask = 0;
  int32_t tgb = 0;
  if (PAT && a.desc) {
    constexpr int W = H / 64, DW = kDescWords<R>;
    typedef int iv __attribute__((ext_vector_type(DW)));
    const iv d = *reinterpret_cast<const iv*>(a.desc + DW * s);
    off = (int64_t)d[0] * H;
    lraw = d[1];
    const int wi = (lane * R) / 64;
#pragma unroll
    for (int i = 0; i < W; ++i) {
      const uint64_t mw = (uint64_t)(uint32_t)d[4 + 2 * i] | ((uint64_t)(uint32_t)d[5 + 2 * i] << 32);
      if (i == 0 || wi == i) dmask = mw;
    }
  } else if (PK == 4 && a.desc) {
    typedef int i4v __attribute__((ext_vector_type(4)));
    const i4v d = *reinterpret_cast<const i4v*>(a.desc + 4 * s);
    off = (int64_t)d[0] * H;
    lraw = d[1];
    tgb = d[2];
  } else {
    off = a.soff[s];
    lraw = a.slen[s];
  }
  const int len = PAT ? (lraw & 0xff) : (PK == 4 ? (lraw & kTriLen) : lraw);
  bool ok[R];
  if (PAT) {
    const uint64_t m = a.desc ? dmask : a.mask[s * (H / 64) + (lane * R) / 64];
#pragma unroll
    for (int r = 0; r < R; ++r) ok[r] = ((m >> ((lane * R + r) & 63)) & 1ull) && (row0 + r < a.nrows);
  } else {
#pragma unroll
    for (int r = 0; r < R; ++r) ok[r] = row0 + (int64_t)r * rs < a.nrows;
    if (a.sflags && a.sflags[s]) {
      const uint64_t m = a.lmask[s * (H / 64) + (lane * R) / 64];
#pragma unroll
      for (int r = 0; r < R; ++r) ok[r] = ok[r] && !((m >> ((lane * R + r) & 63)) & 1ull);
    }
  }
  int64_t orow[R];
#pragma unroll
  for (int r = 0; r < R; ++r) {
    const int64_t i = row0 + (int64_t)r * rs;
    orow[r] = ok[r] ? (a.rowmap ? (int64_t)a.rowmap[i] : i) : 0;
    if constexpr (PK == 4) {
      if (orow[r] < 0) {
        ok[r] = false;
        orow[r] = 0;
      }
    }
  }

  T acc[R];
#pragma unroll
  for (int r = 0; r < R; ++r) {
    if (BMODE == 0) {
      acc[r] = zero_of<T>();
    } else {
      T yo = zero_of<T>();
      if (ok[r]) yo = a.y[a.ymap ? (int64_t)a.ymap[orow[r]] : orow[r]];
      acc[r] = (BMODE == 2) ? yo * a.beta : yo;
    }
  }

  const Pack<T, R>* __restrict__ vp = reinterpret_cast<const Pack<T, R>*>(a.val + off) + lane;
  const bool tb = (a.flags & SPMV_TAILB) != 0;
  const bool pf = (a.flags & SPMV_PRODA) != 0;
  if constexpr (PK == 1) {
    const int32_t* pat = a.pat + (int64_t)(lraw >> 9) * a.kmax;
    bool tri_done = false;
    if constexpr (R > 1 && !SH) {
      if ((lraw & 0x100) && (a.flags & SPMV_XPAIR)) {
        if (a.flags & SPMV_NT) rows_pattern_tri<T, R, ALPHA, true>(acc, pat, vp, len, xs, row0, ok, a.alpha, pf);
        else rows_pattern_tri<T, R, ALPHA, false>(acc, pat, vp, len, xs, row0, ok, a.alpha, pf);
        tri_done = true;
      }
    }
    if (tri_done) {
    } else if (a.flags & SPMV_XPAIR) {
      if (a.flags & SPMV_NT) rows_pattern<T, R, ALPHA, true, U, true, SH>(acc, pat, vp, len, xs, row0, ok, a.alpha, pf, tb);
      else rows_pattern<T, R, ALPHA, false, U, true, SH>(acc, pat, vp, len, xs, row0, ok, a.alpha, pf, tb);
    } else {
      if (a.flags & SPMV_NT) rows_pattern<T, R, ALPHA, true, U, false, SH>(acc, pat, vp, len, xs, row0, ok, a.alpha, pf, tb);
      else rows_pattern<T, R, ALPHA, false, U, false, SH>(acc, pat, vp, len, xs, row0, ok, a.alpha, pf, tb);
    }
  } else if constexpr (PK == 3) {
    const S16Pack<R>* __restrict__ cp = reinterpret_cast<const S16Pack<R>*>(a.col16 + off) + lane;
    const int32_t gb = a.gbase[s];
    int32_t rw[R];
#pragma unroll
    for (int r = 0; r < R; ++r) rw[r] = (int32_t)row0 + r * kD16RowStride<R>;
    if (a.flags & SPMV_NT) rows_d16<T, R, ALPHA, true, U, SH, kIdsAhead<T, R>>(acc, cp, vp, len, xs, a.alpha, pf, tb, rw, gb);
    else rows_d16<T, R, ALPHA, false, U, SH, kIdsAhead<T, R>>(acc, cp, vp, len, xs, a.alpha, pf, tb, rw, gb);
  } else if constexpr (PK == 4) {
    const S16Pack<R>* __restrict__ cp = reinterpret_cast<const S16Pack<R>*>(a.col16 + off) + lane;
    const int32_t gb = a.desc ? tgb : a.gbase[s];
    int32_t rw[R];
#pragma unroll
    for (int r = 0; r < R; ++r) rw[r] = (int32_t)orow[r];
    if (lraw & kTriSlice) {
      bool packed = false;
      if constexpr (R == 2) {
        using XS = XSrc<T, XV>;
        const bool tp = sizeof(T) == 4 && (a.flags & SPMV_TPACK);
        packed = true;
        if (lraw & kTriPair) {
          const uint16_t* cs = (const uint16_t*)a.col16 + off;
          if constexpr (sizeof(T) == 4) {
            if (tp) rows_t16_pair<T, ALPHA, XS, true>(acc, cs, vp, len, xs, a.alpha, pf, rw[0], gb);
            else rows_t16_pair<T, ALPHA, XS, false>(acc, cs, vp, len, xs, a.alpha, pf, rw[0], gb);
          } else {
            rows_t16_pair<T, ALPHA, XS, false>(acc, cs, vp, len, xs, a.alpha, pf, rw[0], gb);
          }
        } else {
          packed = false;
        }
      }
      if (packed) {
      } else if (a.flags & SPMV_NT) rows_t16_tri<T, R, ALPHA, true>(acc, cp, vp, len, xs, a.alpha, pf, rw, gb);
      else rows_t16_tri<T, R, ALPHA, false>(acc, cp, vp, len, xs, a.alpha, pf, rw, gb);
    } else {
      if (a.flags & SPMV_NT) rows_d16<T, R, ALPHA, true, U, SH, kIdsAhead<T, R>>(acc, cp, vp, len, xs, a.alpha, pf, tb, rw, gb);
      else rows_d16<T, R, ALPHA, false, U, SH, kIdsAhead<T, R>>(acc, cp, vp, len, xs, a.alpha, pf, tb, rw, gb);
    }
  } else {
    const IPack<R>* __restrict__ cp = reinterpret_cast<const IPack<R>*>(a.col + off) + lane;
    if (a.flags & SPMV_NT) rows_int32<T, R, ALPHA, true, U, SH, kIdsAhead<T, R>>(acc, cp, vp, len, xs, a.alpha, pf, tb);
    else rows_int32<T, R, ALPHA, false, U, SH, kIdsAhead<T, R>>(acc, cp, vp, len, xs, a.alpha, pf, tb);
  }

  T un[R];
  if constexpr (XV) {
    if (main_rows) cg_rows_update<T, R, true>(a, xs, row0, rs, xalpha, xpend, un);
  }
  if (a.dotp) {
    using DA = typename DAcc<T>::type;
    DA part = zero_of<DA>();
#pragma unroll
    for (int r = 0; r < R; ++r) {
      T uv;
      if constexpr (XV) uv = main_rows ? un[r] : xs.get(orow[r]);
      else uv = a.dotu[orow[r]];
      if (ok[r]) part = part + dacc(cdot(uv, acc[r]));
    }
#pragma unroll
    for (int d = 32; d >= 1; d >>= 1) part = part + shfl_down_acc(part, d);
    if (lane == 0) reinterpret_cast<DA*>(a.dotp)[a.dot_base + s] = part;
  }

  bool all = true;
#pragma unroll
  for (int r = 0; r < R; ++r) all = all && ok[r];
  if (all && !a.ymap && !a.rowmap && !il) {
    Pack<T, R> o;
#pragma unroll
    for (int r = 0; r < R; ++r) o.v[r] = acc[r];
    if constexpr (sizeof(Pack<T, R>) == 16) {
      if (a.flags & SPMV_YNT) {
        spmv_u32x4 w;
        __builtin_memcpy(&w, &o, 16);
        __builtin_nontemporal_store(w, reinterpret_cast<spmv_u32x4*>(a.y + row0));
      } else {
        *reinterpret_cast<Pack<T, R>*>(a.y + row0) = o;
      }
    } else {
      *reinterpret_cast<Pack<T, R>*>(a.y + row0) = o;
    }
// ... 217 lines not shown
      if ((knobs().spmv_flags & SPMV_SHORT) && a.maxlen <= 8)
        hipLaunchKernelGGL((k_spmv_sell<T, R, false, 0, 8, PAT, true, true>), dim3(blocks), dim3(256), 0, st, a);
      else
        hipLaunchKernelGGL((k_spmv_sell<T, R, false, 0, 8, PAT, false, true>), dim3(blocks), dim3(256), 0, st, a);
      return;
    }
  }
  if ((knobs().spmv_flags & SPMV_SHORT) && a.maxlen <= 8)
    hipLaunchKernelGGL((k_spmv_sell<T, R, ALPHA, BMODE, 8, PAT, true>), dim3(blocks), dim3(256), 0, st, a);
  else
    hipLaunchKernelGGL((k_spmv_sell<T, R, ALPHA, BMODE, 8, PAT>), dim3(blocks), dim3(256), 0, st, a);
}

template <typename T, int R, int PAT>
static void launch_ab(const SpmvArgs<T>& a, bool has_alpha, int bmode, hipStream_t st) {
  if (!has_alpha) {
    if (bmode == 0) launch_t<T, R, false, 0, PAT>(a, st);
    else if (bmode == 1) launch_t<T, R, false, 1, PAT>(a, st);
    else launch_t<T, R, false, 2, PAT>(a, st);
  } else {
    if (bmode == 0) launch_t<T, R, true, 0, PAT>(a, st);
    else if (bmode == 1) launch_t<T, R, true, 1, PAT>(a, st);
    else launch_t<T, R, true, 2, PAT>(a, st);
  }
}

template <typename T>
static SpmvArgs<T> make_args(int which, int64_t nwork, const int32_t* list, const pa_mat* A, const void* x,
                             void* y, const int32_t* ymap, const void* alpha, const void* beta, void* dotp,
                             const SpmvPart* cgp = nullptr) {
  SpmvArgs<T> a{};
  if (cgp && cgp->cg) {
    a.xu = (decltype(a.xu))((const T*)cgp->xu);
    a.un = (decltype(a.un))((T*)cgp->un);
    a.xacc = (decltype(a.xacc))((T*)cgp->xacc);
    a.cg = (decltype(a.cg))(cgp->cg);
  }
  a.dotu = (decltype(a.dotu))((const T*)x);
  a.dotp = dotp;
  a.dot_base = which == 2 ? A->nslices : which == 5 ? A->nslices + A->s_nslices : 0;
  a.nwork = nwork;
  a.list = (decltype(a.list))(list);
  a.x = (decltype(a.x))((const T*)x);
  a.nx = A->ncols_lids;
  a.y = (decltype(a.y))((T*)y);
  a.ymap = (decltype(a.ymap))(ymap);
  a.alpha = *(const T*)alpha;
  a.beta = *(const T*)beta;
  a.flags = knobs().spmv_flags | (A->csr ? SPMV_PRODA : 0) | (which == 5 && (A->t_pack & 1) ? SPMV_TPACK : 0);
  a.xcd_chunk = knobs().spmv_xcd_chunk >= 0 ? knobs().spmv_xcd_chunk : A->xcd_auto;
  a.maxlen = which == 0   ? A->maxlen_pat
             : which == 2 ? A->maxlen_side
             : which == 1 ? ((knobs().spmv_format == 1 && A->has_pat) ? A->maxlen_pm_int : A->maxlen_all)
             : which == 4 ? A->maxlen_d16
             : which == 5 ? std::max(A->maxlen_t, 9)
                          : INT32_MAX;
  if (which == 5) {
    a.soff = (decltype(a.soff))(A->d_t_off);
    a.slen = (decltype(a.slen))(A->d_t_len);
    a.col16 = (decltype(a.col16))(A->d_t_col16);
    a.gbase = (decltype(a.gbase))(A->d_t_gbase);
    a.val = (decltype(a.val))((const T*)A->d_t_val);
    a.rowmap = (decltype(a.rowmap))(A->d_t_rowmap);
    a.nrows = A->t_nrows;
    if (knobs().spmv_flags & SPMV_DESC) a.desc = (decltype(a.desc))(A->d_t_desc);
  } else if (which == 2) {
    a.soff = (decltype(a.soff))(A->d_s_off);
    a.slen = (decltype(a.slen))(A->d_s_len);
    a.col = (decltype(a.col))(A->d_s_col);
    a.val = (decltype(a.val))((const T*)A->d_s_val);
    a.rowmap = (decltype(a.rowmap))(A->d_s_rowmap);
    a.nrows = A->s_nrows;
  } else {
    a.soff = (decltype(a.soff))(A->d_slice_off);
    a.col = (decltype(a.col))(A->d_col);
    a.val = (decltype(a.val))((const T*)A->d_val);
    a.nrows = A->nrows;
    if (which == 0) {
      a.slen = (decltype(a.slen))(A->d_plen);
      a.pat = (decltype(a.pat))(A->d_pat);
      a.mask = (decltype(a.mask))(A->d_mask);
      a.kmax = A->kmax;
      if (knobs().spmv_flags & SPMV_DESC) a.desc = (decltype(a.desc))(A->d_pdesc);
      if (A->d_uval && a.desc) {
        a.uval = (decltype(a.uval))((const T*)A->d_uval);
        a.uK = A->uK;
        for (int e = 0; e < 8; ++e) a.upat[e] = A->upat[e];
      }
    } else {
      a.slen = (decltype(a.slen))(A->d_slice_len);
      if (which == 4) {
        a.col16 = (decltype(a.col16))(A->d_col16);
        a.gbase = (decltype(a.gbase))(A->d_gbase);
      }
    }
  }
  if (which == 1) {
    a.sflags = (decltype(a.sflags))(A->d_sflags);
    a.lmask = (decltype(a.lmask))(A->d_lmask);
    if (A->d_col16 && A->R == 4 && !(knobs().spmv_format == 1 && A->has_pat)) a.ilv = (decltype(a.ilv))(A->d_kind);
  }
  return a;
}

template <typename T, int R>
static void launch_which(int which, int64_t nwork, const int32_t* list, const pa_mat* A, const void* x,
                         void* y, const int32_t* ymap, bool has_alpha, int bmode, const void* alpha,
                         const void* beta, void* dotp, hipStream_t st, const SpmvPart* cgp) {
  const SpmvArgs<T> a = make_args<T>(which, nwork, list, A, x, y, ymap, alpha, beta, dotp, cgp);
  if (which == 0) launch_ab<T, R, 1>(a, has_alpha, bmode, st);
  else if (which == 4) launch_ab<T, R, 3>(a, has_alpha, bmode, st);
  else if (which == 5) {
    if constexpr (R <= 2) launch_ab<T, R, 4>(a, has_alpha, bmode, st);
  } else launch_ab<T, R, 0>(a, has_alpha, bmode, st);
}

template <typename T, int R>
static void group_which(int which, int np, const SpmvPart* parts, bool has_alpha, int bmode, const void* alpha,
                        const void* beta, hipStream_t st) {
  SpmvGroup<T> g{};
  g.tail0 = PA_GROUP_MAX + 1;
  auto flush = [&]() {
    if (g.np == 0) return;
    if (which == 0 || which == 6) launch_group_ab<T, R, 1>(g, has_alpha, bmode, st);
    else if (which == 4) launch_group_ab<T, R, 3>(g, has_alpha, bmode, st);
    else if (which == 5) {
      if constexpr (R <= 2) launch_group_ab<T, R, 4>(g, has_alpha, bmode, st);
    }
    else launch_group_ab<T, R, 0>(g, has_alpha, bmode, st);
    g = SpmvGroup<T>{};
    g.tail0 = PA_GROUP_MAX + 1;
  };
  for (int i = 0; i < np; ++i) {
    const SpmvPart& q = parts[i];
    if (q.nwork <= 0) continue;
    const int kind = which == 6 ? (q.side ? 2 : 0) : which;
    if (which == 6 && q.side && g.tail0 > g.np) g.tail0 = g.np;
    const int32_t* list = q.list;
    if ((knobs().spmv_flags & SPMV_IDLIST) && list && kind != 2 && kind != 5 && q.nwork == q.A->nslices) list = nullptr;
    g.a[g.np] = make_args<T>(kind, q.nwork, list, q.A, q.x, q.y, q.ymap, alpha, beta, q.dotp, &q);
    g.start[g.np + 1] = g.start[g.np] + q.nwork;
    if (++g.np == PA_GROUP_MAX) flush();
  }
  flush();
}

#define PA_DT_DECL(k)                                                                                          \
  void spmv_group_##k(int which, int np, const SpmvPart* parts, bool has_alpha, int bmode, const void* alpha,  \
                      const void* beta, hipStream_t st);                                                        \
  int spmv_merged_##k(int n, const int* which, const SpmvPart* parts, bool has_alpha, int bmode,              \
                      const void* alpha, const void* beta, pa_ctx* owner, hipStream_t st);                     \
  void spmv_long_##k(const pa_mat* A, const void* x, void* y, const int32_t* ymap, bool has_alpha, int bmode,  \
                     const void* alpha, const void* beta, void* dotp, int64_t dot_base, hipStream_t st);       \
  void spmv_part_##k(int which, int64_t nwork, const int32_t* list, const pa_mat* A, const void* x, void* y,  \
                     const int32_t* ymap, bool has_alpha, int bmode, const void* alpha, const void* beta,     \
                     void* dotp, hipStream_t st, const SpmvPart* cgp);
PA_DT_DECL(0)
PA_DT_DECL(1)
PA_DT_DECL(2)
PA_DT_DECL(3)
#undef PA_DT_DECL
#if defined(PA_SPMV_DT)
#if PA_SPMV_DT == 0
using DtT = float;
constexpr int kDtR = 4;
#elif PA_SPMV_DT == 1
// ... 1085 lines not shown
  }
}

template <int R>
__device__ __forceinline__ int64_t main_slot0(int64_t soff, int w) {
  return kInterleaveD16<R> ? soff + (int64_t)(w & 63) * R + (w >> 6) : soff + (int64_t)(w / R) * R + (w % R);
}

template <int R>
__global__ void k_t_rowinfo(int64_t n, const int32_t* __restrict__ rows, int H, const int64_t* __restrict__ soff,
                            const int32_t* __restrict__ slen, const int32_t* __restrict__ col, int64_t noids,
                            int32_t* __restrict__ info) {
  const int64_t i = blockIdx.x * (int64_t)blockDim.x + threadIdx.x;
  if (i >= n) return;
  const int64_t row = rows[i], s = row / H;
  const int64_t b = main_slot0<R>(soff[s], (int)(row - s * H));
  const int L = slen[s];
  int len = 0;
  bool reg = true, ghost = false, pad = false, bad = false;
  int32_t prev = 0;
  for (int k = 0; k < L; ++k) {
    const int32_t c = col[b + (int64_t)k * 64 * R];
    if (c < 0) { pad = true; continue; }
    if (pad) bad = true;
    if (len % 3 != 0 && c != prev + 1) reg = false;
    ghost = ghost || c >= noids;
    prev = c;
    ++len;
  }
  reg = reg && len > 0 && len % 3 == 0;
  info[i] = len | (reg ? 1 << 28 : 0) | (ghost ? 1 << 29 : 0) | (bad ? 1 << 30 : 0);
}

template <int R>
__global__ void k_t_pairinfo(int64_t n, const int32_t* __restrict__ rows, int H, const int64_t* __restrict__ soff,
                             const int32_t* __restrict__ slen, const int32_t* __restrict__ col,
                             int32_t* __restrict__ pairable) {
  const int64_t i = blockIdx.x * (int64_t)blockDim.x + threadIdx.x;
  if (i >= n) return;
  int32_t ok = 0;
  if (i + 1 < n && rows[i + 1] == rows[i] + 1) {
    const int64_t ra = rows[i], rb = ra + 1, sa = ra / H, sb = rb / H;
    const int64_t ba = main_slot0<R>(soff[sa], (int)(ra - sa * H)), bb = main_slot0<R>(soff[sb], (int)(rb - sb * H));
    const int La = slen[sa], Lb = slen[sb];
    ok = 1;
    for (int k = 0; k < max(La, Lb); ++k) {
      const int32_t ca = k < La ? col[ba + (int64_t)k * 64 * R] : -1;
      const int32_t cb = k < Lb ? col[bb + (int64_t)k * 64 * R] : -1;
      if (ca < 0 && cb < 0) break;
      if (ca < 0 || cb != ca + 1) {
        ok = 0;
        break;
      }
    }
  }
  pairable[i] = ok;
}

template <typename E, int R>
__global__ void k_u_fill(int64_t ns, int H, int K, const int32_t* __restrict__ kind, const int64_t* __restrict__ soff,
                         const int32_t* __restrict__ plen, const int32_t* __restrict__ emap,
                         const E* __restrict__ val, E* __restrict__ uval) {
  const int64_t i = blockIdx.x * (int64_t)blockDim.x + threadIdx.x;
  if (i >= ns * 8 * 64) return;
  const int64_t s = i / (8 * 64);
  const int k = (int)((i / 64) % 8), l = (int)(i % 64);
  if (kind[s] != 1) return;
  const int32_t lraw = plen[s];
  if (k >= (lraw & 0xff)) return;
  const int e = emap[(lraw >> 9) * 8 + k];
#pragma unroll
  for (int r = 0; r < R; ++r)
    uval[s * H * K + ((int64_t)e * 64 + l) * R + r] = val[soff[s] + ((int64_t)k * 64 + l) * R + r];
}

void launch_u_fill(const pa_mat* A, hipStream_t st) {
  const int64_t n = A->nslices * 8 * 64;
  if (n == 0 || !A->d_uval) return;
  hipLaunchKernelGGL((k_u_fill<double, 2>), dim3((unsigned)((n + 255) / 256)), dim3(256), 0, st, A->nslices, A->H,
                     A->uK, A->d_kind, A->d_slice_off, A->d_plen, A->d_uemap, (const double*)A->d_val,
                     (double*)A->d_uval);
}

void launch_t_pairinfo(const pa_mat* A, int64_t n, const int32_t* rows, int32_t* pairable, hipStream_t st) {
  if (n == 0) return;
  const dim3 g((unsigned)((n + 255) / 256)), b(256);
#define PA_TPI(RR) hipLaunchKernelGGL(k_t_pairinfo<RR>, g, b, 0, st, n, rows, A->H, A->d_slice_off, A->d_slice_len, \
                                      A->d_col, pairable)
  switch (A->R) {
    case 1: PA_TPI(1); break;
    case 2: PA_TPI(2); break;
    case 4: PA_TPI(4); break;
  }
#undef PA_TPI
}

template <int R>
__global__ __launch_bounds__(256) void k_t_gbase(int64_t ns, int64_t nrows, int H, const int32_t* __restrict__ rowlen,
                                                 const int64_t* __restrict__ src, const int32_t* __restrict__ col,
                                                 int64_t noids, int32_t* __restrict__ gbase, int32_t* __restrict__ ok) {
  const int64_t s = (int64_t)blockIdx.x * 4 + (threadIdx.x >> 6);
  if (s >= ns) return;
  const int lane = threadIdx.x & 63;
  int32_t gmin = INT32_MAX, gmax = -1;
  for (int w = lane; w < H; w += 64) {
    const int64_t i = s * H + w;
    if (i >= nrows) break;
    for (int k = 0; k < rowlen[i]; ++k) {
      const int32_t c = col[src[i] + (int64_t)k * 64 * R];
      if (c >= noids) { gmin = min(gmin, c); gmax = max(gmax, c); }
    }
  }
  for (int d = 32; d >= 1; d >>= 1) {
    gmin = min(gmin, __shfl_xor(gmin, d, 64));
    gmax = max(gmax, __shfl_xor(gmax, d, 64));
  }
  if (lane == 0) {
    gbase[s] = gmin == INT32_MAX ? 0 : gmin;
    ok[s] = gmin == INT32_MAX || (int64_t)gmax - gmin <= 32766;
  }
}

__device__ __forceinline__ int64_t t_code_slot(int64_t d, int g, int ntri, int lane, int r, int R, bool packed,
                                               int B) {
  const int b = g / B, i = g % B, nq = 4 * (B / 4);
  if (!packed || B * (b + 1) > ntri) return d + ((int64_t)g * 64 + lane) * R + r;
  const int64_t bb = d + (int64_t)b * B * 64 * R;
  return i < nq ? bb + (int64_t)(i / 4) * 4 * 64 * R + (int64_t)lane * 4 * R + (i % 4) * R + r
                : bb + (int64_t)i * 64 * R + (int64_t)lane * R + r;
}

template <typename E, int R>
__global__ void k_t_fill(int64_t nrows, int H, const int32_t* __restrict__ rowmap, const int32_t* __restrict__ rowlen,
                         const int64_t* __restrict__ src, const int64_t* __restrict__ toff,
                         const int32_t* __restrict__ tlen, const int32_t* __restrict__ gbase,
                         const int32_t* __restrict__ col, const E* __restrict__ val, int64_t noids, bool codes,
                         int pack, uint16_t* __restrict__ col16, E* __restrict__ tval) {
  const int64_t i = blockIdx.x * (int64_t)blockDim.x + threadIdx.x;
  if (i >= nrows) return;
  const int64_t ts = i / H;
  const int w = (int)(i - ts * H), lane = w & 63, r = w >> 6;
  if (rowmap[i] < 0) return;
  const int32_t lraw = tlen[ts];
  const int L = lraw & kTriLen;
  const bool tri = (lraw & kTriSlice) != 0, pair = (lraw & kTriPair) != 0;
  constexpr int B = sizeof(E) == 4 ? 9 : 4;
  const int n = rowlen[i];
  const int64_t b = src[i], d = toff[ts];
  const int32_t oid = rowmap[i], gb = gbase[ts];
  for (int k = 0; k < L; ++k) {
    const int64_t sk = b + (int64_t)k * 64 * R;
    E v;
    __builtin_memset(&v, 0, sizeof(E));
    if (k < n) v = val[sk];
    if ((pack & 1) && pair && sizeof(E) == 4) {
      const int64_t tb = d + (int64_t)(k / 3) * 3 * 64 * R;
      const int j = k % 3;
      tval[j < 2 ? tb + (int64_t)lane * 2 * R + j * R + r : tb + 2 * 64 * R + (int64_t)lane * R + r] = v;
    } else {
      tval[d + ((int64_t)k * 64 + lane) * R + r] = v;
    }
    if (!codes || (tri && k % 3 != 0) || (pair && r != 0)) continue;
    uint16_t q = 0xFFFFu;
    if (k < n) {
      const int32_t c = col[sk];
      q = c < noids ? (uint16_t)((uint32_t)(c - oid) & 0x7FFFu) : (uint16_t)(0x8000u | (uint32_t)(c - gb));
// ... 87 lines not shown
```

### partitionedarrays.jl_amd/device.py

```python
from __future__ import annotations

import ctypes as C
import sys

import numpy as np

from . import _lib
from .backends import DistributedBackend, PData, SequentialBackend


class PartContext:

    def __init__(self, device: int, part: int, nparts: int, share_with=None):
        h = C.c_void_p()
        if share_with is not None:
            _lib.call("pa_ctx_create_shared", part, nparts, share_with.h, C.byref(h))
        else:
            _lib.call("pa_ctx_create", device, part, nparts, C.byref(h))
        self.h = h
        self.device = device
        self.part = part
        self.nparts = nparts

    def sync(self):
# ... 348 lines not shown
        if not (len(I) == len(J) == len(V)):
            raise ValueError("sparse: I, J and V must have the same length")
        colptr = np.empty((nrows_lids if csr_bi is not None else ncols_lids) + 1, dtype=np.int64) if pattern else None
        rowval = np.empty(max(1, len(I)), dtype=np.int64) if pattern else None
        nnz = C.c_int64(0)
        h = C.c_void_p()
        ptrs = (colptr.ctypes.data_as(C.POINTER(C.c_int64)) if pattern else None,
                rowval.ctypes.data_as(C.POINTER(C.c_int64)) if pattern else None)
        if csr_bi is None:
            _lib.call("pa_mat_from_coo", ctx.h, _lib.DTYPES[V.dtype], ib, 1 if ids_global else 0, nrows_lids,
                      ncols_lids, len(I), I.ctypes.data_as(C.c_void_p), J.ctypes.data_as(C.c_void_p),
                      V.ctypes.data_as(C.c_void_p), rows_idx.h, cols_idx.h, C.byref(nnz), *ptrs, C.byref(h))
        else:
            _lib.call("pa_mat_from_coo_csr", ctx.h, _lib.DTYPES[V.dtype], ib, 1 if ids_global else 0, int(csr_bi),
                      nrows_lids, ncols_lids, len(I), I.ctypes.data_as(C.c_void_p), J.ctypes.data_as(C.c_void_p),
                      V.ctypes.data_as(C.c_void_p), rows_idx.h, cols_idx.h, C.byref(nnz), *ptrs, C.byref(h))
        M = DeviceMatrix(h, ctx, V.dtype)
        M.csc_nnz = nnz.value
        if not pattern:
            return M, None, None
        return M, colptr, rowval[:nnz.value].copy()

    @staticmethod
    def from_dcoo(coo: DeviceCOO, rows_idx: DeviceIndex, cols_idx: DeviceIndex, nrows_lids, ncols_lids,
                  ids_global=True, pattern=True, csr_bi=None):
        n = len(coo)
        colptr = np.empty((nrows_lids if csr_bi is not None else ncols_lids) + 1, dtype=np.int64) if pattern else None
        rowval = np.empty(max(1, n), dtype=np.int64) if pattern else None
        nnz = C.c_int64(0)
        h = C.c_void_p()
        ptrs = (colptr.ctypes.data_as(C.POINTER(C.c_int64)) if pattern else None,
                rowval.ctypes.data_as(C.POINTER(C.c_int64)) if pattern else None)
        if csr_bi is None:
            _lib.call("pa_mat_from_dcoo", coo.h, 1 if ids_global else 0, nrows_lids, ncols_lids, rows_idx.h,
                      cols_idx.h, C.byref(nnz), *ptrs, C.byref(h))
        else:
            _lib.call("pa_mat_from_dcoo_csr", coo.h, 1 if ids_global else 0, int(csr_bi), nrows_lids, ncols_lids,
                      rows_idx.h, cols_idx.h, C.byref(nnz), *ptrs, C.byref(h))
        M = DeviceMatrix(h, coo.ctx, coo.dtype)
        M.csc_nnz = nnz.value
        if not pattern:
            return M, None, None
        return M, colptr, rowval[:nnz.value].copy()

    def set_values(self, nzval):
        nzval = np.ascontiguousarray(nzval, dtype=self.dtype)
        _lib.call("pa_mat_set_values", self.h, nzval.ctypes.data_as(C.c_void_p))

    def fillstored(self, v):
        buf, ptr = _lib.scalar_buf(v, self.dtype)
        _lib.call("pa_mat_fillstored", self.h, ptr)
        del buf

    def get_values(self):
        n = getattr(self, "csc_nnz", None)
        if n is None:
            raise _lib.PAError("matrix was not built from a CSC pattern")
        a = np.empty(n, dtype=self.dtype)
        _lib.call("pa_mat_get_values", self.h, a.ctypes.data_as(C.c_void_p))
        return a

    def cg_choice(self) -> int:
        v = C.c_int(-1)
        _lib.call("pa_mat_cg_choice", self.h, C.byref(v))
        return v.value

    def info(self):
        v = [C.c_int64() for _ in range(5)]
        _lib.call("pa_mat_info", self.h, *[C.byref(x) for x in v])
        d = dict(zip(["nrows", "nnz", "slots", "nslices", "nslices_interior"], [x.value for x in v]))
        f = [C.c_int64() for _ in range(4)]
        _lib.call("pa_mat_format_info", self.h, *[C.byref(x) for x in f])
        d.update(zip(["pattern_slices", "regular_rows", "side_rows", "side_slots"], [x.value for x in f]))
        dd = C.c_int64()
        _lib.call("pa_mat_delta16_info", self.h, C.byref(dd))
        d["delta16_slices"] = dd.value
        t = [C.c_int64() for _ in range(4)]
        _lib.call("pa_mat_triple_info", self.h, *[C.byref(x) for x in t])
        d.update(zip(["triple_sell_slices", "triple_sell_rows", "tri_slices", "tri_rows"], [x.value for x in t]))
        pr = [C.c_int64() for _ in range(2)]
        if hasattr(_lib.lib(), "pa_mat_pair_info"):
            _lib.call("pa_mat_pair_info", self.h, *[C.byref(x) for x in pr])
        d.update(zip(["pair_slices", "pair_rows"], [x.value for x in pr]))
        lr = [C.c_int64() for _ in range(2)]
        _lib.call("pa_mat_long_rows", self.h, *[C.byref(x) for x in lr])
        d.update(zip(["long_rows", "long_nnz"], [x.value for x in lr]))
        d.update(self.traffic())
        return d

    def device_ptrs(self):
        out = (C.c_uint64 * 8)()
        _lib.call("pa_mat_device_ptrs", self.h, out)
        return dict(zip(["val", "col", "slice_off", "plen", "pat", "mask", "s_val", "s_col"], list(out)))

    def traffic(self):
        t = [C.c_int64() for _ in range(3)]
        _lib.call("pa_mat_traffic", self.h, *[C.byref(x) for x in t])
        return dict(zip(["value_bytes", "index_bytes", "meta_bytes"], [x.value for x in t]))

    def __del__(self):
        try:
            if getattr(self, "h", None) and _lib._lib is not None and not sys.is_finalizing():
                _lib._lib.pa_mat_destroy(self.h)
        except Exception:
            pass
```

Baseline: 6597.

## Read constant-coefficient pattern slices from a deduplicated value-row table

Adds build-time detection of pattern slices whose regular rows all hold bit-identical values. Their distinct value rows are deduplicated on the host into a small table, and each slice's id is written into a spare descriptor word. The SpMV kernel then loads one coefficient per entry from that table through the constant address space instead of streaming per-row value slots, cutting value traffic for constant-coefficient stencils. In exchange, matrix builds and value writes gain a detection kernel, a host copy and a hash pass, and the traffic accounting changes.

```diff
diff --git a/include/pa_hip.h b/include/pa_hip.h
--- a/include/pa_hip.h
+++ b/include/pa_hip.h
@@ -128,6 +128,7 @@
 int pa_mat_triple_info(const pa_mat* A, int64_t* t_slices, int64_t* t_rows, int64_t* tri_slices,
                        int64_t* tri_rows);
 int pa_mat_pair_info(const pa_mat* A, int64_t* pair_slices, int64_t* pair_rows);
+int pa_mat_const_info(const pa_mat* A, int64_t* const_slices, int64_t* value_rows);
 
 int pa_mat_device_ptrs(const pa_mat* A, uint64_t out[8]);
 
diff --git a/partitionedarrays.jl_amd/_lib.py b/partitionedarrays.jl_amd/_lib.py
--- a/partitionedarrays.jl_amd/_lib.py
+++ b/partitionedarrays.jl_amd/_lib.py
@@ -88,6 +88,7 @@
     "pa_mat_delta16_info": [_p, _i64p],
     "pa_mat_triple_info": [_p, _i64p, _i64p, _i64p, _i64p],
     "pa_mat_pair_info": [_p, _i64p, _i64p],
+    "pa_mat_const_info": [_p, _i64p, _i64p],
     "pa_mat_long_rows": [_p, _i64p, _i64p],
     "pa_mat_stencil": [_p, C.c_int, C.c_int, _i64p, _i64p, _i64p, C.c_int64, _i32p, C.POINTER(C.c_double), C.c_int, C.POINTER(_p)],
     "pa_spmv_all": [C.c_int, C.POINTER(_p), C.POINTER(_p), C.POINTER(_p), C.POINTER(_p), C.POINTER(_p), C.POINTER(_p), _p, _p],
diff --git a/partitionedarrays.jl_amd/csrc/pa_api.cpp b/partitionedarrays.jl_amd/csrc/pa_api.cpp
--- a/partitionedarrays.jl_amd/csrc/pa_api.cpp
+++ b/partitionedarrays.jl_amd/csrc/pa_api.cpp
@@ -54,7 +54,8 @@
      223,  1,  1,  1,  1,
      65536,  2,  1,  0,  1,
      1,  0,  1,  0,  -1,  1,
-     1,  1,  1,  0,  7,  1};
+     1,  1,  1,  0,  7,  1,
+     1};
 int coo_compress(int dtype, int index_bytes, int64_t m, int64_t ncols, int64_t n, const void* dI, const void* dJ,
                  const void* dV, int csr, int64_t* nu_out, int32_t** crow, int32_t** ccol, void** cval,
                  int64_t** colptr, hipStream_t st, hipError_t* err_out);
@@ -111,6 +112,8 @@
 void launch_t_rowinfo(const pa_mat* A, int64_t n, const int32_t* rows, int64_t noids, int32_t* info, hipStream_t st);
 void launch_t_pairinfo(const pa_mat* A, int64_t n, const int32_t* rows, int32_t* pairable, hipStream_t st);
 void launch_u_fill(const pa_mat* A, hipStream_t st);
+void launch_const_detect(const pa_mat* A, int32_t* flag, void* rows, hipStream_t st);
+void launch_const_apply(const pa_mat* A, const int32_t* cid, hipStream_t st);
 void launch_t_gbase(const pa_mat* A, int64_t noids, int32_t* ok, hipStream_t st);
 void launch_t_fill(const pa_mat* A, int64_t noids, bool codes, hipStream_t st);
 void launch_t_check(const pa_mat* A, unsigned* bad, hipStream_t st);
@@ -324,6 +327,81 @@
   for (int e = 0; e < 8; ++e) A->upat[e] = e < K ? U[e] : 0;
   launch_u_fill(A, st);
   HIPC(hipGetLastError());
+  return 0;
+}
+
+void free_const(pa_mat* A) {
+  dev_free(A->d_cval);
+  A->d_cval = nullptr;
+  A->ncval = A->cval_cap = A->nconst_slices = 0;
+  A->h_cid.clear();
+}
+
+int build_const(pa_mat* A, hipStream_t st) {
+  const int64_t ns = A->nslices, K = A->kmax;
+  if (!A->has_pat || !A->d_pdesc || A->npattern_slices == 0 || ns == 0) return 0;
+  if (!knobs().spmv_const) {
+    if (A->nconst_slices > 0) {
+      std::vector<int32_t> zero(ns, 0);
+      int32_t* d_cid = nullptr;
+      if (dev_upload(&d_cid, zero)) return -1;
+      launch_const_apply(A, d_cid, st);
+      HIPC(hipGetLastError());
+      HIPC(hipStreamSynchronize(st));
+      dev_free(d_cid);
+    }
+    free_const(A);
+    return 0;
+  }
+  const size_t S = dtype_size(A->dtype);
+  int32_t *d_flag = nullptr, *d_cid = nullptr;
+  void* d_rows = nullptr;
+  HIPC(hipMalloc((void**)&d_flag, ns * 4));
+  HIPC(hipMalloc(&d_rows, (size_t)ns * K * S));
+  launch_const_detect(A, d_flag, d_rows, st);
+  HIPC(hipGetLastError());
+  std::vector<int32_t> flag(ns);
+  std::vector<unsigned char> rows((size_t)ns * K * S);
+  HIPC(hipMemcpyAsync(flag.data(), d_flag, ns * 4, hipMemcpyDeviceToHost, st));
+  HIPC(hipMemcpyAsync(rows.data(), d_rows, (size_t)ns * K * S, hipMemcpyDeviceToHost, st));
+  HIPC(hipStreamSynchronize(st));
+  dev_free(d_flag);
+  dev_free(d_rows);
+  std::vector<unsigned char> table;
+  std::unordered_map<std::string, int32_t> ids;
+  A->h_cid.assign(ns, 0);
+  A->nconst_slices = 0;
+  for (int64_t s = 0; s < ns; ++s) {
+    if (A->h_kind[s] != 1 || !flag[s]) continue;
+    const size_t nb = (size_t)A->h_plen[s] * S;
+    std::string key(reinterpret_cast<const char*>(&rows[(size_t)s * K * S]), nb);
+    auto it = ids.find(key);
+    int32_t id;
+    if (it == ids.end()) {
+      id = (int32_t)ids.size();
+      table.insert(table.end(), key.begin(), key.end());
+      table.resize((size_t)(id + 1) * K * S, 0);
+      ids.emplace(std::move(key), id);
+    } else {
+      id = it->second;
+    }
+    A->h_cid[s] = id + 1;
+    ++A->nconst_slices;
+  }
+  A->ncval = (int64_t)ids.size();
+  if (A->ncval > A->cval_cap) {
+    dev_free(A->d_cval);
+    A->d_cval = nullptr;
+    A->cval_cap = 0;
+    HIPC(hipMalloc(&A->d_cval, (size_t)A->ncval * K * S));
+    A->cval_cap = A->ncval;
+  }
+  if (A->ncval) HIPC(hipMemcpyAsync(A->d_cval, table.data(), (size_t)A->ncval * K * S, hipMemcpyHostToDevice, st));
+  if (dev_upload(&d_cid, A->h_cid)) return -1;
+  launch_const_apply(A, d_cid, st);
+  HIPC(hipGetLastError());
+  HIPC(hipStreamSynchronize(st));
+  dev_free(d_cid);
   return 0;
 }
 
@@ -721,6 +799,7 @@
     HIPC(hipStreamSynchronize(st));
   }
   A->has_pat = true;
+  if (build_const(A, st)) return -1;
   return 0;
 }
 
@@ -1261,6 +1340,11 @@
      "spmv_uniform: Float64 pattern slices whose patterns (<= 7 entries) fit one union U (FD7; matrices built "
      "afterwards): 1 = a copy of their values at slice * H * |U| in U's entry order, so the short-row tail "
      "launch issues its value and x loads before the slice descriptor arrives (default), 0 = off"},
+    {"spmv_const", &Knobs::spmv_const, nullptr, 0, 1, 0,
+     "spmv_const: 1 = a pattern slice whose regular rows all hold the same values, entry for entry and bit for "
+     "bit (constant-coefficient stencils), reads them from a table of the distinct value rows instead of its "
+     "value slots (detected when a matrix is built and whenever its values are written; default), 0 = no "
+     "detection, every slice streams its values"},
     {"spmv_side_tail", &Knobs::side_tail, nullptr, 0, 1, 0,
      "spmv_side_tail: per-kind launches without a halo in flight (big single parts): 1 = the side rows (<= 8 "
      "entries) run as the trailing waves of the pattern launch (default: FE27 256^3 -0.4 %, profiles/r05/o/), "
@@ -2729,11 +2813,13 @@
     launch_u_fill(A, st);
     HIPC(hipGetLastError());
   }
+  if (build_const(A, st)) return -1;
   return 0;
 }
 
 int pa_mat_set_values(pa_mat* A, const void* nzval) {
   CHECK_ARG(A && nzval, "null argument");
+  TuneScope ts(A->ctx);
   if (load_nz_map(A)) return -1;
   HIPC(hipSetDevice(A->ctx->device));
   const size_t S = dtype_size(A->dtype);
@@ -2750,6 +2836,7 @@
 
 int pa_mat_fillstored(pa_mat* A, const void* v) {
   CHECK_ARG(A && v, "null argument");
+  TuneScope ts(A->ctx);
   HIPC(hipSetDevice(A->ctx->device));
   const int64_t nv = nvals(A);
   if (nv) launch_fill(A->dtype, nv, 0, nullptr, A->d_val, v, A->ctx->s_main);
@@ -2845,6 +2932,7 @@
     dev_free(p);
   free_triple_sell(A);
   free_uniform(A);
+  free_const(A);
   delete A;
   return 0;
 }
@@ -2882,6 +2970,13 @@
   return 0;
 }
 
+int pa_mat_const_info(const pa_mat* A, int64_t* const_slices, int64_t* value_rows) {
+  CHECK_ARG(A, "null matrix");
+  if (const_slices) *const_slices = A->nconst_slices;
+  if (value_rows) *value_rows = A->ncval;
+  return 0;
+}
+
 int pa_mat_long_rows(const pa_mat* A, int64_t* n_long, int64_t* n_long_nnz) {
   CHECK_ARG(A, "null matrix");
   if (n_long) *n_long = A->n_long;
@@ -2902,10 +2997,15 @@
   const int64_t S = (int64_t)dtype_size(A->dtype), H = A->H, W = H / 64;
   const bool pat = knobs().spmv_format == 1 && A->has_pat;
   const bool split = A->d_bnd_list != nullptr;
+  const bool cst = pat && knobs().spmv_const && (knobs().spmv_flags & 6) == 6 && A->ncval > 0 && !A->h_cid.empty() &&
+                   !A->d_uval;
   int64_t v = 0, ix = 0, m = 0;
   for (int64_t s = 0; s < A->nslices; ++s) {
     const int kd = pat ? A->h_kind[s] : 0;
-    if (kd == 1) {
+    if (kd == 1 && cst && A->h_cid[s]) {
+      v += (int64_t)A->h_plen[s] * S;
+      m += std::max<int64_t>(W * 8 + 8 + 4, 4 * desc_words(A->R)) + 4;
+    } else if (kd == 1) {
       v += (int64_t)(A->d_uval ? A->uK : A->h_plen[s]) * H * S;
       m += std::max<int64_t>(W * 8 + 8 + 4, 4 * desc_words(A->R)) + 4;
     } else if (kd == 3) {
diff --git a/partitionedarrays.jl_amd/csrc/pa_internal.h b/partitionedarrays.jl_amd/csrc/pa_internal.h
--- a/partitionedarrays.jl_amd/csrc/pa_internal.h
+++ b/partitionedarrays.jl_amd/csrc/pa_internal.h
@@ -291,6 +291,7 @@
   int f32_rows;
   int tri_pack;
   int spmv_uniform;
+  int spmv_const;
 };
 const Knobs& knobs();
 struct KnobBind {
@@ -467,6 +468,10 @@
   int32_t* d_uemap = nullptr;
   int uK = 0;
   int32_t upat[8] = {0, 0, 0, 0, 0, 0, 0, 0};
+  void* d_cval = nullptr;
+  int64_t ncval = 0, cval_cap = 0;
+  int64_t nconst_slices = 0;
+  std::vector<int32_t> h_cid;
   int32_t* d_t_gbase = nullptr;
   int32_t* d_t_desc = nullptr;
   int32_t* d_t_rowmap = nullptr;
diff --git a/partitionedarrays.jl_amd/csrc/pa_spmv.hip b/partitionedarrays.jl_amd/csrc/pa_spmv.hip
--- a/partitionedarrays.jl_amd/csrc/pa_spmv.hip
+++ b/partitionedarrays.jl_amd/csrc/pa_spmv.hip
@@ -42,8 +42,10 @@
 
 #if defined(__HIP_DEVICE_COMPILE__)
 #define PA_GLB __attribute__((address_space(1)))
+#define PA_CST __attribute__((address_space(4)))
 #else
 #define PA_GLB
+#define PA_CST
 #endif
 
 template <int BYTES> struct RawOf;
@@ -100,6 +102,7 @@
   const PA_GLB T* uval;
   int uK;
   int32_t upat[8];
+  const PA_GLB T* cval;
 };
 
 template <typename T> struct DAcc { using type = double; };
@@ -599,9 +602,28 @@
   }
 }
 
-template <typename T, int R, bool ALPHA, bool NT, int U, bool XP, bool SH = false, typename XS>
+template <typename T, int R, bool NT, bool CV>
+__device__ __forceinline__ Pack<T, R> pattern_val(const Pack<T, R>* __restrict__ vp, const T* __restrict__ cv, int k) {
+  if constexpr (CV) {
+    const T c = ((const PA_CST T*)cv)[k];
+    Pack<T, R> v;
+#pragma unroll
+    for (int r = 0; r < R; ++r) v.v[r] = c;
+    return v;
+  } else {
+    return ld<NT>(&vp[k * 64]);
+  }
+}
+
+template <bool CV>
+__device__ __forceinline__ int32_t pattern_off(const int32_t* __restrict__ pat, int k) {
+  if constexpr (CV) return ((const PA_CST int32_t*)pat)[k];
+  else return pat[k];
+}
+
+template <typename T, int R, bool ALPHA, bool NT, int U, bool XP, bool SH = false, bool CV = false, typename XS>
 __device__ __forceinline__ void rows_pattern(T (&acc)[R], const int32_t* __restrict__ pat,
-                                             const Pack<T, R>* __restrict__ vp, int len,
+                                             const Pack<T, R>* __restrict__ vp, const T* __restrict__ cv, int len,
                                              const XS& x, int64_t rbase,
                                              const bool (&ok)[R], T alpha, bool pf, bool TB) {
   if (SH) TB = true;
@@ -617,9 +639,9 @@
     int32_t o[U];
     Pack<T, R> v[U];
 #pragma unroll
-    for (int u = 0; u < U; ++u) o[u] = pat[k + u];
-#pragma unroll
-    for (int u = 0; u < U; ++u) v[u] = ld<NT>(&vp[(k + u) * 64]);
+    for (int u = 0; u < U; ++u) o[u] = pattern_off<CV>(pat, k + u);
+#pragma unroll
+    for (int u = 0; u < U; ++u) v[u] = pattern_val<T, R, NT, CV>(vp, cv, k + u);
     T xv[U][R];
     if constexpr (XP && R > 1) {
 #pragma unroll
@@ -645,10 +667,10 @@
     int32_t o[U];
     Pack<T, R> v[U];
 #pragma unroll
-    for (int u = 0; u < U; ++u) o[u] = pat[min(k + u, len - 1)];
+    for (int u = 0; u < U; ++u) o[u] = pattern_off<CV>(pat, min(k + u, len - 1));
 #pragma unroll
     for (int u = 0; u < U; ++u)
-      if (k + u < len) v[u] = ld<NT>(&vp[(k + u) * 64]);
+      if (k + u < len) v[u] = pattern_val<T, R, NT, CV>(vp, cv, k + u);
     T xv[U][R];
     if constexpr (XP && R > 1) {
 #pragma unroll
@@ -676,8 +698,8 @@
     k = len;
   }
   for (; !SH && k < len; ++k) {
-    const int32_t o = pat[k];
-    const Pack<T, R> v = ld<NT>(&vp[k * 64]);
+    const int32_t o = pattern_off<CV>(pat, k);
+    const Pack<T, R> v = pattern_val<T, R, NT, CV>(vp, cv, k);
 #pragma unroll
     for (int r = 0; r < R; ++r) {
       acc[r] = acc[r] + term<ALPHA>(v.v[r], x.get(xb[r] >= 0 ? xb[r] + o : 0), alpha, pf);
@@ -685,9 +707,9 @@
   }
 }
 
-template <typename T, int R, bool ALPHA, bool NT, typename XS>
+template <typename T, int R, bool ALPHA, bool NT, bool CV = false, typename XS>
 __device__ __forceinline__ void rows_pattern_tri(T (&acc)[R], const int32_t* __restrict__ pat,
-                                                 const Pack<T, R>* __restrict__ vp, int len, const XS& x,
+                                                 const Pack<T, R>* __restrict__ vp, const T* __restrict__ cv, int len, const XS& x,
                                                  int64_t rbase, const bool (&ok)[R], T alpha, bool pf) {
   static_assert(R > 1, "runs of R > 1 values");
   bool any = false;
@@ -718,10 +740,10 @@
   for (; k + 3 * TB <= len; k += 3 * TB) {
     int32_t o[TB];
 #pragma unroll
-    for (int t = 0; t < TB; ++t) o[t] = pat[k + 3 * t];
+    for (int t = 0; t < TB; ++t) o[t] = pattern_off<CV>(pat, k + 3 * t);
     Pack<T, R> v[3 * TB];
 #pragma unroll
-    for (int u = 0; u < 3 * TB; ++u) v[u] = ld<NT>(&vp[(k + u) * 64]);
+    for (int u = 0; u < 3 * TB; ++u) v[u] = pattern_val<T, R, NT, CV>(vp, cv, k + u);
     T xv[TB][3][R];
 #pragma unroll
     for (int t = 0; t < TB; ++t) triple(o[t], xv[t]);
@@ -733,10 +755,10 @@
         for (int r = 0; r < R; ++r) acc[r] = acc[r] + term<ALPHA>(v[3 * t + j].v[r], xv[t][j][r], alpha, pf);
   }
   for (; k < len; k += 3) {
-    const int32_t o = pat[k];
+    const int32_t o = pattern_off<CV>(pat, k);
     Pack<T, R> v[3];
 #pragma unroll
-    for (int j = 0; j < 3; ++j) v[j] = ld<NT>(&vp[(k + j) * 64]);
+    for (int j = 0; j < 3; ++j) v[j] = pattern_val<T, R, NT, CV>(vp, cv, k + j);
     T xv[3][R];
     triple(o, xv);
 #pragma unroll
@@ -830,12 +852,14 @@
   int32_t lraw;
   uint64_t dmask = 0;
   int32_t tgb = 0;
+  int32_t cid = 0;
   if (PAT && a.desc) {
     constexpr int W = H / 64, DW = kDescWords<R>;
     typedef int iv __attribute__((ext_vector_type(DW)));
     const iv d = *reinterpret_cast<const iv*>(a.desc + DW * s);
     off = (int64_t)d[0] * H;
     lraw = d[1];
+    cid = d[3];
     const int wi = (lane * R) / 64;
 #pragma unroll
     for (int i = 0; i < W; ++i) {
@@ -897,21 +921,36 @@
   const bool pf = (a.flags & SPMV_PRODA) != 0;
   if constexpr (PK == 1) {
     const int32_t* pat = a.pat + (int64_t)(lraw >> 9) * a.kmax;
-    bool tri_done = false;
-    if constexpr (R > 1 && !SH) {
-      if ((lraw & 0x100) && (a.flags & SPMV_XPAIR)) {
-        if (a.flags & SPMV_NT) rows_pattern_tri<T, R, ALPHA, true>(acc, pat, vp, len, xs, row0, ok, a.alpha, pf);
-        else rows_pattern_tri<T, R, ALPHA, false>(acc, pat, vp, len, xs, row0, ok, a.alpha, pf);
-        tri_done = true;
-      }
-    }
-    if (tri_done) {
-    } else if (a.flags & SPMV_XPAIR) {
-      if (a.flags & SPMV_NT) rows_pattern<T, R, ALPHA, true, U, true, SH>(acc, pat, vp, len, xs, row0, ok, a.alpha, pf, tb);
-      else rows_pattern<T, R, ALPHA, false, U, true, SH>(acc, pat, vp, len, xs, row0, ok, a.alpha, pf, tb);
+    const T* cv = nullptr;
+    if (cid != 0 && a.cval) cv = (const T*)(a.cval + (int64_t)(cid - 1) * a.kmax);
+    const bool tri = R > 1 && !SH && (lraw & 0x100) && (a.flags & SPMV_XPAIR);
+    if (cv) {
+      bool tri_done = false;
+      if constexpr (R > 1 && !SH) {
+        if (tri) {
+          rows_pattern_tri<T, R, ALPHA, false, true>(acc, pat, vp, cv, len, xs, row0, ok, a.alpha, pf);
+          tri_done = true;
+        }
+      }
+      if (!tri_done)
+        rows_pattern<T, R, ALPHA, false, U, true, SH, true>(acc, pat, vp, cv, len, xs, row0, ok, a.alpha, pf, tb);
     } else {
-      if (a.flags & SPMV_NT) rows_pattern<T, R, ALPHA, true, U, false, SH>(acc, pat, vp, len, xs, row0, ok, a.alpha, pf, tb);
-      else rows_pattern<T, R, ALPHA, false, U, false, SH>(acc, pat, vp, len, xs, row0, ok, a.alpha, pf, tb);
+      bool tri_done = false;
+      if constexpr (R > 1 && !SH) {
+        if (tri) {
+          if (a.flags & SPMV_NT) rows_pattern_tri<T, R, ALPHA, true>(acc, pat, vp, cv, len, xs, row0, ok, a.alpha, pf);
+          else rows_pattern_tri<T, R, ALPHA, false>(acc, pat, vp, cv, len, xs, row0, ok, a.alpha, pf);
+          tri_done = true;
+        }
+      }
+      if (tri_done) {
+      } else if (a.flags & SPMV_XPAIR) {
+        if (a.flags & SPMV_NT) rows_pattern<T, R, ALPHA, true, U, true, SH>(acc, pat, vp, cv, len, xs, row0, ok, a.alpha, pf, tb);
+        else rows_pattern<T, R, ALPHA, false, U, true, SH>(acc, pat, vp, cv, len, xs, row0, ok, a.alpha, pf, tb);
+      } else {
+        if (a.flags & SPMV_NT) rows_pattern<T, R, ALPHA, true, U, false, SH>(acc, pat, vp, cv, len, xs, row0, ok, a.alpha, pf, tb);
+        else rows_pattern<T, R, ALPHA, false, U, false, SH>(acc, pat, vp, cv, len, xs, row0, ok, a.alpha, pf, tb);
+      }
     }
   } else if constexpr (PK == 3) {
     const S16Pack<R>* __restrict__ cp = reinterpret_cast<const S16Pack<R>*>(a.col16 + off) + lane;
@@ -1295,6 +1334,8 @@
       a.mask = (decltype(a.mask))(A->d_mask);
       a.kmax = A->kmax;
       if (knobs().spmv_flags & SPMV_DESC) a.desc = (decltype(a.desc))(A->d_pdesc);
+      if (A->ncval > 0 && a.desc && knobs().spmv_const && (knobs().spmv_flags & SPMV_XPAIR))
+        a.cval = (decltype(a.cval))((const T*)A->d_cval);
       if (A->d_uval && a.desc) {
         a.uval = (decltype(a.uval))((const T*)A->d_uval);
         a.uK = A->uK;
@@ -2546,6 +2587,88 @@
                      (double*)A->d_uval);
 }
 
+struct u128 {
+  uint64_t a, b;
+};
+__device__ __forceinline__ bool same_bits(uint32_t x, uint32_t y) { return x == y; }
+__device__ __forceinline__ bool same_bits(uint64_t x, uint64_t y) { return x == y; }
+__device__ __forceinline__ bool same_bits(u128 x, u128 y) { return x.a == y.a && x.b == y.b; }
+
+template <typename E, int R>
+__global__ __launch_bounds__(256) void k_const_detect(int64_t ns, int64_t nrows, int kmax,
+                                                      const int32_t* __restrict__ kind,
+                                                      const int64_t* __restrict__ soff,
+                                                      const int32_t* __restrict__ plen,
+                                                      const uint64_t* __restrict__ mask, const E* __restrict__ val,
+                                                      int32_t* __restrict__ flag, E* __restrict__ rows) {
+  constexpr int H = 64 * R;
+  const int lane = threadIdx.x & 63;
+  const int64_t s = (int64_t)blockIdx.x * 4 + (threadIdx.x >> 6);
+  if (s >= ns) return;
+  if (kind[s] != 1) {
+    if (lane == 0) flag[s] = 0;
+    return;
+  }
+  const int len = plen[s] & 0xff;
+  const uint64_t m = mask[s * (H / 64) + (lane * R) / 64];
+  bool ok[R];
+  int first = -1;
+#pragma unroll
+  for (int r = 0; r < R; ++r) {
+    ok[r] = ((m >> ((lane * R + r) & 63)) & 1ull) && (s * H + (int64_t)lane * R + r < nrows);
+    if (ok[r] && first < 0) first = r;
+  }
+  const uint64_t have = __ballot(first >= 0);
+  if (have == 0) {
+    if (lane == 0) flag[s] = 0;
+    return;
+  }
+  const int fl = __ffsll((unsigned long long)have) - 1;
+  const int fr = __shfl(first, fl, 64);
+  const E* v = val + soff[s];
+  bool differs = false;
+  for (int k = 0; k < len; ++k) {
+    const E ref = v[((int64_t)k * 64 + fl) * R + fr];
+#pragma unroll
+    for (int r = 0; r < R; ++r)
+      if (ok[r] && !same_bits(v[((int64_t)k * 64 + lane) * R + r], ref)) differs = true;
+    if (lane == 0) rows[s * kmax + k] = ref;
+  }
+  const uint64_t bad = __ballot(differs);
+  if (lane == 0) flag[s] = bad == 0 ? 1 : 0;
+}
+
+void launch_const_detect(const pa_mat* A, int32_t* flag, void* rows, hipStream_t st) {
+  const int64_t ns = A->nslices;
+  if (ns == 0) return;
+  const dim3 g((unsigned)((ns + 3) / 4)), b(256);
+#define PA_CD(E, RR)                                                                                            \
+  hipLaunchKernelGGL((k_const_detect<E, RR>), g, b, 0, st, ns, A->nrows, A->kmax, A->d_kind, A->d_slice_off,    \
+                     A->d_plen, A->d_mask, (const E*)A->d_val, flag, (E*)rows)
+  switch (A->dtype) {
+    case PA_F32:
+      if (A->R == 2) PA_CD(uint32_t, 2);
+      else PA_CD(uint32_t, 4);
+      break;
+    case PA_F64: PA_CD(uint64_t, 2); break;
+    case PA_C64: PA_CD(uint64_t, 2); break;
+    case PA_C128: PA_CD(u128, 1); break;
+  }
+#undef PA_CD
+}
+
+__global__ void k_const_apply(int64_t ns, int DW, const int32_t* __restrict__ cid, int32_t* __restrict__ desc) {
+  const int64_t s = blockIdx.x * (int64_t)blockDim.x + threadIdx.x;
+  if (s < ns) desc[DW * s + 3] = cid[s];
+}
+
+void launch_const_apply(const pa_mat* A, const int32_t* cid, hipStream_t st) {
+  const int64_t ns = A->nslices;
+  if (ns == 0 || !A->d_pdesc) return;
+  hipLaunchKernelGGL(k_const_apply, dim3((unsigned)((ns + 255) / 256)), dim3(256), 0, st, ns, desc_words(A->R), cid,
+                     A->d_pdesc);
+}
+
 void launch_t_pairinfo(const pa_mat* A, int64_t n, const int32_t* rows, int32_t* pairable, hipStream_t st) {
   if (n == 0) return;
   const dim3 g((unsigned)((n + 255) / 256)), b(256);
diff --git a/partitionedarrays.jl_amd/device.py b/partitionedarrays.jl_amd/device.py
--- a/partitionedarrays.jl_amd/device.py
+++ b/partitionedarrays.jl_amd/device.py
@@ -454,6 +454,10 @@
         if hasattr(_lib.lib(), "pa_mat_pair_info"):
             _lib.call("pa_mat_pair_info", self.h, *[C.byref(x) for x in pr])
         d.update(zip(["pair_slices", "pair_rows"], [x.value for x in pr]))
+        cr = [C.c_int64() for _ in range(2)]
+        if hasattr(_lib.lib(), "pa_mat_const_info"):
+            _lib.call("pa_mat_const_info", self.h, *[C.byref(x) for x in cr])
+        d.update(zip(["const_slices", "const_value_rows"], [x.value for x in cr]))
         lr = [C.c_int64() for _ in range(2)]
         _lib.call("pa_mat_long_rows", self.h, *[C.byref(x) for x in lr])
         d.update(zip(["long_rows", "long_nnz"], [x.value for x in lr]))
```

Result: slower. 2025 (-69.3%).
